# genetronhealth/uvc

Measured on AMD Instinct MI355X. Metric: pileup positions scored/sec at 300x depth, higher is better.
Workload: dtype int32

## Files before the change

### uvc_amd/csrc/uvc_device.h

```cpp
#ifndef UVC_DEVICE_H
#define UVC_DEVICE_H

#include <hip/hip_runtime.h>
#include <stdint.h>
#include "uvcgpu.h"

#define NSYM UVC_NUM_SYMBOLS
#define NBUCKETS 16
#define SQR_QUAL_DIV 32
#define MAX_INSERT_SIZE 2000
#define MAX_STR_N_BASES 100
#define UVC_MAXEV 8
#define UVC_DIGEST_MAX_VOTES (1 << 22)

enum { C_MATCH = 0, C_INS = 1, C_DEL = 2, C_REF_SKIP = 3, C_SOFT_CLIP = 4, C_HARD_CLIP = 5, C_PAD = 6, C_EQUAL = 7, C_DIFF = 8 };

struct AlnRec {
    int32_t pos, rend, mpos, isize;
    int32_t flag, mapq, dflag, l_qseq;
    int64_t seq_off;
    int64_t qbase;
    int64_t cigar_off;
    int64_t table_off;
    int64_t item_off;
    int64_t gap_off;
    int32_t n_cigar, kind;
    int32_t xm1500, go1500;
    int32_t bm1500[5];
    int32_t clip_cnt;
    int32_t nogap_penal, indel_penal;
    int32_t lclip_len, rclip_len;
    int32_t lclip_oplen, rclip_oplen;
    int32_t lclip_q;
    int32_t m_index;
    int32_t frag, fs;
    int32_t id;
    int32_t n_mutc;
    int64_t baq_pos, baq_last, baq2_last;
};

struct FastRec {
    int32_t pos, rend, qb_lo, aln;
    int32_t fmd, isize, mpos, xm1500;
    int32_t bmv, xbv, bm4c, clips;
    int32_t baq_pos, baq_last, baq2_last, ext;
};

struct FragRec {
    int32_t aln_beg, aln_end;
    int32_t beg, end;
    int32_t fs, strand, dflag, normMQ;
    int32_t n_cov, n_near;
    int32_t singleton;
    int32_t stat_kind;
};

struct FsRec {
    int32_t frag_beg, frag_end;
    int32_t beg, end;
    int32_t strand, dflag, fam, generic;
    int64_t work_off;
    int32_t l2r_end_median, r2l_end_median, nsb_min, nsb_max;
    int32_t other_fs;
    int32_t pad_;
};
static_assert(sizeof(FsRec) == 64, "k_fam_p4d fetches a unit record as four 16-byte words per lane");

struct Item { int32_t epos; uint8_t sym, flags ; uint16_t val; uint16_t dist, indel_len; int32_t pad2; };
static_assert(sizeof(Item) == 16, "Item");

struct MisItem { int32_t rank, epos, symval; };

struct FragUnit { int32_t v[12]; };
enum { UVC_FSUM_LCNT = 0 , UVC_FSUM_LTA = 5, UVC_FSUM_LTB, UVC_FSUM_LSING, UVC_FSUM_LMQ, UVC_FSUM_BDP, UVC_FSUM_BTA, UVC_FSUM_BTB, UVC_FSUM_BMQ, UVC_FSUM_N };
struct FragFast {
    int32_t beg, end, fi, flags;
    int32_t pos0, rend0, pos1, rend1;
    int32_t qb0, qb1, nogap0, nogap1;
    int32_t sq, n_cov, n_near, pad_;
    int32_t bpos0, brend0, bqb0, sp0;
    int32_t bpos1, brend1, bqb1, sp1;
};

struct AlnGap {
    int32_t epos, sym;
    int32_t len, qpos;
    int32_t weight, aln;
    int32_t mark, pad_;
};
struct GapRow { int32_t x, sym, len, ev; int64_t seq_off; int32_t cnt[8]; };
struct GapWork {
    AlnGap *ev; int32_t n_ev;
    unsigned long long *ckey, *ckey_s, *cval, *cval_s;
    unsigned long long *ikey, *ikey_s, *ival, *ival_s;
    int32_t inc_cap; int32_t *n_inc;
    GapRow *rows; int32_t *n_rows; uint8_t *seq; unsigned long long *seq_len; int64_t seq_cap;
    int32_t *maj;
    void *sort_tmp; size_t sort_tmp_bytes;
};

struct Contrib { uint8_t bsym_p1 , lmask ; uint16_t bval; uint16_t lval[8]; uint16_t pad_[2]; };
static_assert(sizeof(Contrib) == 24, "Contrib rows are zero-filled as bytes and indexed as 24-byte records");

struct HapWork { int32_t *cand, *cand_off, *cand_cap; int32_t *n_cand; unsigned long long *total; int32_t *events; };

struct DevParams { UvcParams P; };

struct RegionDev {
    int32_t beg, end; int64_t npos;
    const uint8_t *refsym;
    int32_t *rtr;
    const int64_t *baq;
    int32_t *prep32; int64_t *prep64; int32_t *thres;
    int32_t *seg32; int64_t *seg64; int32_t *vq; int32_t *bqsum;
    int32_t *frag; int32_t *fam; int32_t *faminfo32; int64_t *faminfo64; int32_t *duplex;
    int32_t *bucket;
    const uint8_t *bases; const uint8_t *quals; const uint32_t *cigars;
    const uint16_t *bq; uint32_t bq_bytes;
    AlnRec *alns; int32_t n_alns;
    int32_t n_fast;
    FastRec *frec;
    int32_t p2_off[5];
    FastRec *frec2; int32_t n_fast2; int32_t max_p2_span;
    const int32_t *complex_ids; int32_t n_complex;
    FragRec *frags; int32_t n_frags;
    int32_t *frag_nmut; int32_t *frag_mut;
    const int32_t *sweep_frags; int32_t n_sweep;
    int32_t *overflow_frags; int32_t *n_overflow;
    const int32_t *frag_sorted;
    const int32_t *frag_rank;
    int32_t frag_off[3];
    FragFast *ffast;
    FragUnit *ffast_u;
    int32_t *win; int32_t nwin;
    int32_t *fsum;
    FsRec *fss; int32_t n_fs;
    const int32_t *generic_fs; int32_t n_generic_fs; int64_t n_generic_work;
    const int32_t *generic_sorted; int32_t max_unit_span;
    uint8_t *p5flag;
    uint8_t *dirty; int32_t ndblk;
    uint32_t *occ;
    uint32_t *fam_digest;
    Contrib *table;
    int32_t *ir_list;
    Item *items; int32_t *item_cnt;
    MisItem *mis; int32_t *mis_cnt; int32_t mis_cap;
    unsigned long long *mis_total;
    int32_t max_aln_span, max_frag_span;
    int32_t any_amplicon;
    int32_t frag32;
    int32_t max_frag_depth;
    int32_t *err;
    GapWork gap;
};

#define DEV __device__ __forceinline__

DEV int imin(int a, int b) { return a < b ? a : b; }
DEV int imax(int a, int b) { return a > b ? a : b; }
DEV int64_t lmin(int64_t a, int64_t b) { return a < b ? a : b; }
DEV int64_t lmax(int64_t a, int64_t b) { return a > b ? a : b; }
DEV int64_t nnminus(int64_t a, int64_t b) { return a > b ? a - b : 0; }
DEV int ibetween(int v, int a, int b) { return imin(imax(a, v), b); }
DEV bool is_ins(int s) { return s == UVC_LINK_I3P || s == UVC_LINK_I2 || s == UVC_LINK_I1; }
DEV bool is_del(int s) { return s == UVC_LINK_D3P || s == UVC_LINK_D2 || s == UVC_LINK_D1; }
DEV bool is_subst(int s) { return s <= UVC_BASE_NN; }
DEV bool symbols_mutated(int ref, int alt) {
    if (alt <= UVC_BASE_NN) return ref != alt && ref < UVC_BASE_N && alt < UVC_BASE_N;
    return alt != UVC_LINK_M && alt != UVC_LINK_NN;
}
DEV int cig_op(uint32_t c) { return (int)(c & 0xF); }
DEV int cig_len(uint32_t c) { return (int)(c >> 4); }

#define P32(R, f, x) ((R).prep32[(size_t)(f) * (R).npos + (x)])
#define P64(R, f, x) ((R).prep64[(size_t)(f) * (R).npos + (x)])
#define TH(R, f, x) ((R).thres[(size_t)(f) * (R).npos + (x)])
#define S32(R, f, s, x) ((R).seg32[((size_t)(f) * NSYM + (s)) * (R).npos + (x)])
#define S64(R, f, s, x) ((R).seg64[((size_t)(f) * NSYM + (s)) * (R).npos + (x)])
#define VQP(R, f, s, x) ((R).vq[((size_t)(f) * NSYM + (s)) * (R).npos + (x)])
#define BQS(R, s, x) ((R).bqsum[(size_t)(s) * (R).npos + (x)])
#define FRP(R, st, f, s, x) ((R).frag[(((size_t)(st) * UVC_NFRAG + (f)) * NSYM + (s)) * (R).npos + (x)])
#define FAP(R, st, f, s, x) ((R).fam[(((size_t)(st) * UVC_NFAM + (f)) * NSYM + (s)) * (R).npos + (x)])
#define FIP(R, f, s, x) ((R).faminfo32[((size_t)(f) * NSYM + (s)) * (R).npos + (x)])
#define FI64P(R, f, s, x) ((R).faminfo64[((size_t)(f) * NSYM + (s)) * (R).npos + (x)])
#define DUP(R, f, s, x) ((R).duplex[((size_t)(f) * NSYM + (s)) * (R).npos + (x)])
#define BKP(R, st, s, b, x) ((R).bucket[((((size_t)(st) * NSYM + (s)) * NBUCKETS) + (b)) * (R).npos + (x)])
#define RTRP(R, f, x) ((R).rtr[(size_t)(f) * (R).npos + (x)])
#define BAQ1(R, p) ((R).baq[(p) - (R).beg])
#define BAQ2(R, p) ((R).baq[(R).npos + (p) - (R).beg])

DEV int cov_PREP32(const RegionDev &R, int plane, int64_t x) { return P32(R, plane, x); }
DEV int cov_FRAG(const RegionDev &R, int plane, int64_t x) {
    int v = 0;
#pragma unroll
    for (int sd = 0; sd < 2; sd++)
#pragma unroll
        for (int s = UVC_BASE_A; s <= UVC_BASE_NN; s++) v += FRP(R, sd, plane, s, x);
    return v;
}
DEV int cov_FAM(const RegionDev &R, int plane, int64_t x) {
    int v = 0;
#pragma unroll
    for (int sd = 0; sd < 2; sd++)
#pragma unroll
        for (int s = UVC_BASE_A; s <= UVC_BASE_NN; s++) v += FAP(R, sd, plane, s, x);
    return v;
}
DEV int cov_DUPLEX(const RegionDev &R, int plane, int64_t x) {
    int v = 0;
#pragma unroll
    for (int s = UVC_BASE_A; s <= UVC_BASE_NN; s++) v += DUP(R, plane, s, x);
    return v;
}

#define UVC_DIRTY_SHIFT 12
DEV bool sym_always_filled(int s) { return s < UVC_BASE_NN || s == UVC_LINK_M; }
DEV void occ_mark(const RegionDev &R, int s, int64_t x) { if (s != UVC_LINK_M && s != (int)R.refsym[x] && !((R.occ[x] >> s) & 1u)) atomicOr(&R.occ[x], 1u << s); }
DEV void mark_sym(const RegionDev &R, int s, int64_t x) { occ_mark(R, s, x); if (!sym_always_filled(s)) R.dirty[(size_t)s * R.ndblk + (x >> UVC_DIRTY_SHIFT)] = 1; }
DEV void mark_fi(const RegionDev &R, int s, int64_t x) { R.dirty[((size_t)NSYM + s) * R.ndblk + (x >> UVC_DIRTY_SHIFT)] = 1; }
DEV void mark_dup(const RegionDev &R, int s, int64_t x) { occ_mark(R, s, x); R.dirty[((size_t)2 * NSYM + s) * R.ndblk + (x >> UVC_DIRTY_SHIFT)] = 1; }

DEV void add64(int64_t *p, int64_t v) { atomicAdd((unsigned long long *)p, (unsigned long long)v); }
DEV void add_own(int32_t *p, int v) { __hip_atomic_fetch_add(p, v, __ATOMIC_RELAXED, __HIP_MEMORY_SCOPE_WORKGROUP); }
DEV void add64_own(int64_t *p, int64_t v) { __hip_atomic_fetch_add((unsigned long long *)p, (unsigned long long)v, __ATOMIC_RELAXED, __HIP_MEMORY_SCOPE_WORKGROUP); }

template <int STRIDE> struct LdsCounts {
    int *p;
    DEV int &operator[](int s) const { return p[s * STRIDE]; }
};

template <class Arr>
// ... 83 lines not shown
```

### uvc_amd/csrc/uvc_gap.hip

```cpp
#include <algorithm>
#include <cstring>
#include <hip/hip_runtime.h>
#include <rocprim/device/device_radix_sort.hpp>
#include <stdint.h>
#include "uvc_launch.h"

extern "C" size_t uvc_gap_sort_tmp_bytes(size_t n) {
    size_t bytes = 0;
    unsigned long long *k = nullptr;
    rocprim::radix_sort_pairs(nullptr, bytes, k, k, k, k, n, 0, 64, (hipStream_t)0);
    return bytes;
}

extern "C" int uvc_gap_sort(void *tmp, size_t tmp_bytes, const unsigned long long *kin, unsigned long long *kout, const unsigned long long *vin, unsigned long long *vout,
                            size_t n, int end_bit, hipStream_t s) {
    if (n == 0) return 0;
    return rocprim::radix_sort_pairs(tmp, tmp_bytes, kin, kout, vin, vout, n, 0, (unsigned)end_bit, s) == hipSuccess ? 0 : -1;
}

__global__ void __launch_bounds__(256) k_keys_pos_cls(const int32_t *pos, const int32_t *cls, int32_t beg, int shift, int64_t n, uint32_t *key, uint32_t *val) {
    const int64_t i = (int64_t)blockIdx.x * blockDim.x + threadIdx.x;
    if (i >= n) return;
    key[i] = ((uint32_t)(pos[i] - beg) | ((uint32_t)cls[i] << shift)); val[i] = (uint32_t)i;
}
__global__ void __launch_bounds__(256) k_gather4(const uint32_t *perm, int64_t n, const int32_t *a0, const int32_t *a1, const int32_t *a2, const int32_t *a3,
                                                 int32_t *o0, int32_t *o1, int32_t *o2, int32_t *o3) {
    const int64_t i = (int64_t)blockIdx.x * blockDim.x + threadIdx.x;
    if (i >= n) return;
    const int64_t j = (int64_t)perm[i];
    o0[i] = a0[j]; o1[i] = a1[j]; o2[i] = a2[j]; o3[i] = a3[j];
}
__global__ void __launch_bounds__(256) k_rank_from_sorted(const uint32_t *perm, int64_t n, int64_t n_first, int32_t *out_ids, int32_t *rank) {
    const int64_t k = (int64_t)blockIdx.x * blockDim.x + threadIdx.x;
    if (k >= n) return;
    const int32_t id = (int32_t)perm[k];
    if (out_ids && k < n_first) out_ids[k] = id;
    if (rank) rank[id] = (k < n_first ? (int32_t)k : -1);
}
extern "C" size_t uvc_sort32_tmp_bytes(size_t n) {
    size_t bytes = 0;
    uint32_t *k = nullptr;
    rocprim::radix_sort_pairs(nullptr, bytes, k, k, k, k, std::max<size_t>(n, 1), 0, 32, (hipStream_t)0);
    return bytes;
}
extern "C" int uvc_sort_by_pos_cls(const int32_t *d_pos, const int32_t *d_cls, int32_t beg, int pos_bits, int cls_bits, int64_t n, uint32_t *work , void *tmp, size_t tmp_bytes, hipStream_t s) {
    if (n <= 0) return 0;
    if (pos_bits < 1 || cls_bits < 0 || pos_bits + cls_bits > 32) return -1;
    uint32_t *key = work, *key_s = work + n, *val = work + 2 * n, *val_s = work + 3 * n;
    hipLaunchKernelGGL(k_keys_pos_cls, dim3((unsigned)((n + 255) / 256)), dim3(256), 0, s, d_pos, d_cls, beg, pos_bits, n, key, val);
    return rocprim::radix_sort_pairs(tmp, tmp_bytes, key, key_s, val, val_s, (size_t)n, 0, (unsigned)(pos_bits + cls_bits), s) == hipSuccess ? 0 : -1;
}
extern "C" void uvc_launch_gather4(const uint32_t *perm, int64_t n, const int32_t *a0, const int32_t *a1, const int32_t *a2, const int32_t *a3, int32_t *o0, int32_t *o1, int32_t *o2, int32_t *o3, hipStream_t s) {
    if (n > 0) hipLaunchKernelGGL(k_gather4, dim3((unsigned)((n + 255) / 256)), dim3(256), 0, s, perm, n, a0, a1, a2, a3, o0, o1, o2, o3);
}
extern "C" void uvc_launch_rank_from_sorted(const uint32_t *perm, int64_t n, int64_t n_first, int32_t *out_ids, int32_t *rank, hipStream_t s) {
    if (n > 0) hipLaunchKernelGGL(k_rank_from_sorted, dim3((unsigned)((n + 255) / 256)), dim3(256), 0, s, perm, n, n_first, out_ids, rank);
}

struct ColGroups { const char *base[UVC_NUM_FIELD_GROUPS]; int32_t first_col[UVC_NUM_FIELD_GROUPS + 1]; int32_t elem[UVC_NUM_FIELD_GROUPS]; };
__global__ void __launch_bounds__(256) k_gather_columns(ColGroups G, int64_t npos, const int32_t *xs, int64_t n, int32_t n_cols, long long *out) {
    const int64_t t = (int64_t)blockIdx.x * blockDim.x + threadIdx.x;
    if (t >= n * n_cols) return;
    const int64_t i = t / n_cols; const int32_t c = (int32_t)(t - i * n_cols);
    const int64_t x = xs[i];
    long long v = 0;
    if (x >= 0 && x < npos) {
        int g = 0;
        while (g + 1 < UVC_NUM_FIELD_GROUPS && c >= G.first_col[g + 1]) g++;
        const int64_t at = (int64_t)(c - G.first_col[g]) * npos + x;
        v = (G.elem[g] == 8) ? ((const long long *)G.base[g])[at] : (long long)((const int32_t *)G.base[g])[at];
    }
    out[t] = v;
}
extern "C" void uvc_launch_gather_columns(const char *const *base, const int32_t *first_col, const int32_t *elem, int64_t npos, const int32_t *d_xs, int64_t n, long long *d_out, hipStream_t s) {
    ColGroups G;
    for (int g = 0; g < UVC_NUM_FIELD_GROUPS; g++) { G.base[g] = base[g]; G.first_col[g] = first_col[g]; G.elem[g] = elem[g]; }
    G.first_col[UVC_NUM_FIELD_GROUPS] = first_col[UVC_NUM_FIELD_GROUPS];
    const int32_t n_cols = first_col[UVC_NUM_FIELD_GROUPS];
    const int64_t total = n * n_cols;
    if (total > 0) hipLaunchKernelGGL(k_gather_columns, dim3((unsigned)((total + 255) / 256)), dim3(256), 0, s, G, npos, d_xs, n, n_cols, d_out);
}
```

### uvc_amd/csrc/uvc_host.cpp

```cpp
#include "uvc_launch.h"
#include "uvc_host.h"
#include "uvc_alloc.h"
#include "uvc_prep.h"
#include "uvc_rtr.h"
#include "uvc_hap.h"
#include "uvc_cpus.h"

#include <algorithm>
#include <chrono>
#include <cmath>
#include <cstring>
#include <memory>
#include <numeric>
#include <string>
#include <thread>
#include <vector>
#define hipMalloc(p, n) uvc_dev_malloc((void **)(p), (n))
#define hipFree(p) uvc_dev_free((void *)(p))

static thread_local std::string g_err;
static int fail(int code, const std::string &msg) { g_err = msg; return code; }
template <class F> static int guarded(const char *what, F &&f) {
    try {
        const int rc = f();
// ... 237 lines not shown
    return 0;
}

static int uvcgpu_region_create_impl(uvcgpu_region_t **out, const UvcParams *params, int32_t tid, int32_t beg, int32_t end, const char *refseq) {
    if (!out || !params || !refseq || end <= beg) return fail(UVCGPU_EINVAL, "bad argument");
    if (const int rc = uvcgpu_params_check(params)) return rc;
    uvcgpu_region *r = new uvcgpu_region();
    memset(&r->prof, 0, sizeof(r->prof));
    memset(&r->R, 0, sizeof(r->R));
    r->P = *params;
    if (hipStreamCreateWithFlags(&r->stream, hipStreamNonBlocking) != hipSuccess) { delete r; return fail(UVCGPU_EDEVICE, "hipStreamCreate failed (no GPU?)"); }
    if (getenv("UVCGPU_ONE_STREAM")) {  }
    else if (hipStreamCreateWithFlags(&r->side, hipStreamNonBlocking) != hipSuccess || hipStreamCreateWithFlags(&r->side3, hipStreamNonBlocking) != hipSuccess || hipEventCreateWithFlags(&r->e_join3, hipEventDisableTiming) != hipSuccess || hipEventCreateWithFlags(&r->e_stat, hipEventDisableTiming) != hipSuccess || hipEventCreateWithFlags(&r->e_alleles, hipEventDisableTiming) != hipSuccess || hipEventCreateWithFlags(&r->e_fork, hipEventDisableTiming) != hipSuccess || hipEventCreateWithFlags(&r->e_join, hipEventDisableTiming) != hipSuccess || hipEventCreateWithFlags(&r->e_fork2, hipEventDisableTiming) != hipSuccess) {
        uvcgpu_region_destroy(r); return fail(UVCGPU_EDEVICE, "hipStreamCreate / hipEventCreate failed");
    }
    if (hipMalloc((void **)&r->R.err, 4) != hipSuccess) { uvcgpu_region_destroy(r); return fail(UVCGPU_ENOMEM, "hipMalloc failed"); }
    const int rc = configure_region(r, tid, beg, end, refseq);
    if (rc) { uvcgpu_region_destroy(r); return rc; }
    *out = r;
    return 0;
}

static int uvcgpu_region_reset_impl(uvcgpu_region_t *r, int32_t tid, int32_t beg, int32_t end, const char *refseq) {
    if (!r || !refseq || end <= beg) return fail(UVCGPU_EINVAL, "bad argument");
    if (stream_open_(r)) return fail(UVCGPU_ESTATE, "reset while a score stream is open");
    HIP_OK(hipStreamSynchronize(r->stream));
    if (r->side) HIP_OK(hipStreamSynchronize(r->side));
    if (r->side3) HIP_OK(hipStreamSynchronize(r->side3));
    free_reads(r);
    return configure_region(r, tid, beg, end, refseq);
}

static void *prep_alloc(void *ctx, size_t bytes, int zero) {
    uvcgpu_region *r = (uvcgpu_region *)ctx;
    char *p = nullptr;
    if (dev_alloc(r, bytes, &p, zero != 0)) return nullptr;
    return p;
}
static int set_reads_on_device(uvcgpu_region_t *r, const UvcReadSoA *d, bool timing, std::chrono::steady_clock::time_point t_prev) {
    auto lap = [&](const char *what) { if (!timing) return; hipStreamSynchronize(r->stream); const auto t = std::chrono::steady_clock::now();
                                       fprintf(stderr, "[uvcgpu set_reads] %-28s %8.2f ms\n", what, std::chrono::duration<double, std::milli>(t - t_prev).count()); t_prev = t; };
    const int64_t n = d->n_reads;
    if (r->npos >= ((int64_t)1 << 29)) return fail(UVCGPU_EUNSUPPORTED, "region longer than 2^29");
    if (d->n_bases >= ((int64_t)1 << 31)) return fail(UVCGPU_EUNSUPPORTED, "more than 2^31 read bases in one region: split the region");
    if (!d->bases && !d->bases4 && d->n_bases > 0) return fail(UVCGPU_EINVAL, "neither bases nor bases4");
    UvcReadSoA dd = *d;
    int32_t *d_bad = nullptr; uint16_t *bq_done = nullptr;
    if (!d->seq_off || !d->cigar_off || !d->bases) {
        int rc0;
        int64_t *so = nullptr, *co = nullptr, *b4o = nullptr; uint8_t *ub = nullptr; char *tmp = nullptr;
        const size_t tb = uvc_prep_compact_tmp_bytes(n);
        if ((rc0 = dev_alloc(r, tb, &tmp)) || (rc0 = dev_alloc(r, 1, &d_bad, true))) return rc0;
        if (!d->seq_off && (rc0 = dev_alloc(r, (size_t)n, &so))) return rc0;
        if (!d->cigar_off && (rc0 = dev_alloc(r, (size_t)n, &co))) return rc0;
        if (!d->bases && ((rc0 = dev_alloc(r, (size_t)n, &b4o)) || (rc0 = dev_alloc(r, (size_t)std::max<int64_t>(d->n_bases, 1), &ub)) || (rc0 = dev_alloc(r, (size_t)std::max<int64_t>(d->n_bases, 1), &bq_done)))) return rc0;
        const int e = uvc_prep_compact(d->l_qseq, d->n_cigar, n, d->n_bases, d->bases ? nullptr : d->bases4, d->n_bases4_bytes, d->quals, so, d->seq_off, co, b4o, ub, bq_done, d_bad, tmp, tb, r->stream);
        if (e) return fail(UVCGPU_EDEVICE, std::string("offset scans: ") + hipGetErrorString((hipError_t)e));
        if (so) dd.seq_off = so;
        if (co) dd.cigar_off = co;
        if (ub) dd.bases = ub;
        d = &dd;
    }
    UvcPrepIn in; memset(&in, 0, sizeof(in));
    in.n_reads = n; in.n_bases = d->n_bases; in.n_cigar_ops = d->n_cigar_ops; in.n_fams = d->n_fams;
    in.pos = d->pos; in.mpos = d->mpos; in.isize = d->isize; in.nm = d->nm; in.l_qseq = d->l_qseq; in.n_cigar = d->n_cigar; in.frag_id = d->frag_id; in.fam_id = d->fam_id;
    in.flag = d->flag; in.mapq = d->mapq; in.fam_strand = d->fam_strand; in.fam_dflag = d->fam_dflag; in.seq_off = d->seq_off; in.cigar_off = d->cigar_off; in.cigars = d->cigars;
    UvcPrepOut o; char msg[256];
    int rc = uvc_prep_reads(&in, &r->P, r->beg, r->end, r->npos, prep_alloc, r, r->stream, &o, msg, (int)sizeof(msg));
    if (rc) return fail(rc, msg);
    lap("nesting + CIGAR facts (device)");
    RegionDev &R = r->R;
    RawReads &W = r->W;
    W.pos = d->pos; W.endpos = o.endpos; W.mpos = d->mpos; W.isize = d->isize; W.flag = d->flag; W.mapq = d->mapq; W.nm = d->nm; W.l_qseq = d->l_qseq; W.n_cigar = d->n_cigar;
    W.frag = o.frag_of; W.fs = o.fs_of; W.dflag = o.dflag_of; W.kind = o.kind; W.seq_off = d->seq_off; W.cigar_off = d->cigar_off; W.table_off = o.table_off; W.item_off = o.item_off; W.gap_off = o.gap_off;
    R.bases = d->bases; R.quals = d->quals; R.cigars = d->cigars;
    R.frag_off[0] = 0; R.frag_off[1] = o.n_frag_strand0; R.frag_off[2] = o.n_frags;
    const int64_t n_simple = o.n_simple; const size_t nf = (size_t)o.n_frags;
    if (bq_done) { R.bq = bq_done; R.bq_bytes = (uint32_t)(d->n_bases * 2); }
    else { uint16_t *b = nullptr; if ((rc = dev_alloc(r, (size_t)std::max<int64_t>(d->n_bases, 1), &b))) return rc; R.bq = b; R.bq_bytes = (uint32_t)(d->n_bases * 2);
      if (!d_bad && (rc = dev_alloc(r, 1, &d_bad, true))) return rc;
      uvc_launch_pack_bq(R.bases, R.quals, b, d->n_bases, d_bad, r->stream); }
    { AlnRec *a; if ((rc = dev_alloc(r, (size_t)n, &a))) return rc; R.alns = a; R.n_alns = (int32_t)n; }
    R.n_fast = (int32_t)n_simple;
    { FastRec *f; if ((rc = dev_alloc(r, (size_t)n_simple, &f))) return rc; R.frec = f; }
    R.complex_ids = o.complex_ids; R.n_complex = o.n_complex;
    R.frags = o.frags; R.n_frags = o.n_frags;
    int pos_bits = 1; while (((int64_t)1 << pos_bits) < r->npos + 1) pos_bits++;
    {
        const size_t nmax = std::max<size_t>(std::max<size_t>((size_t)n, nf), 1);
        int32_t *d_rank, *d_fsorted, *d_frank; uint32_t *work; uint8_t *tmp;
        const size_t tmp_bytes = uvc_sort32_tmp_bytes(nmax);
        if ((rc = dev_alloc(r, (size_t)n, &d_rank)) || (rc = dev_alloc(r, nf, &d_fsorted)) || (rc = dev_alloc(r, nf, &d_frank)) || (rc = dev_alloc(r, 4 * nmax, &work)) || (rc = dev_alloc(r, tmp_bytes + 16, &tmp))) return rc;
        if (uvc_sort_by_pos_cls(W.pos, o.is_complex, r->beg, pos_bits, 1, n, work, tmp, tmp_bytes, r->stream) != 0) return fail(UVCGPU_EDEVICE, "device sort of the alignments failed");
        uvc_launch_rank_from_sorted(work + 3 * n, n, n_simple, nullptr, d_rank, r->stream);
        W.fast_rank = d_rank;
        if (uvc_sort_by_pos_cls(o.frag_beg, o.frag_strand, r->beg, pos_bits, 1, (int64_t)nf, work, tmp, tmp_bytes, r->stream) != 0) return fail(UVCGPU_EDEVICE, "device sort of the fragments failed");
        uvc_launch_rank_from_sorted(work + 3 * nf, (int64_t)nf, (int64_t)nf, d_fsorted, d_frank, r->stream);
        R.frag_sorted = d_fsorted; R.frag_rank = d_frank;
    }
    { FragFast *f; if ((rc = dev_alloc(r, nf, &f, true))) return rc; R.ffast = f; }
    { FragUnit *f; if ((rc = dev_alloc(r, nf, &f, true))) return rc; R.ffast_u = f; }
    R.sweep_frags = o.sweep_frags; R.n_sweep = o.n_sweep;
    { int32_t *q; if ((rc = dev_alloc(r, nf * (size_t)(UVC_MAXEV + 2) + 1, &q, true))) return rc;
      R.frag_nmut = q; R.frag_mut = q + nf; R.overflow_frags = q + nf * (size_t)(UVC_MAXEV + 1); R.n_overflow = q + nf * (size_t)(UVC_MAXEV + 2); }
    R.fss = o.fss; R.n_fs = o.n_fs;
    R.generic_fs = o.generic_fs; R.n_generic_fs = o.n_generic; R.n_generic_work = o.work;
    R.generic_sorted = o.generic_sorted; R.max_unit_span = o.max_unit_span;
    R.frag32 = (getenv("UVCGPU_FRAG32") != nullptr);
    const char *fam_path = getenv("UVCGPU_FAM_PATH");
    const bool generic_forced = (fam_path && !strcmp(fam_path, "generic"));
    R.fam_digest = nullptr;
    if (!generic_forced && o.work > 8 * r->npos && (size_t)o.work * 32 <= ((size_t)48 << 30) && o.max_unit_frags < UVC_DIGEST_MAX_VOTES) {
        uint32_t *q = nullptr; if ((rc = dev_alloc(r, (size_t)o.work * 8, &q))) return rc; R.fam_digest = q;
    }
    if (timing) fprintf(stderr, "[uvcgpu set_reads] %d fragments, %d units, %d generic units, %lld (unit, position) cells, longest unit %d, most fragments in a unit %d, %lld positions, family form %s\n",
                        o.n_frags, o.n_fs, o.n_generic, (long long)o.work, o.max_unit_span, o.max_unit_frags, (long long)r->npos, R.fam_digest ? "digest" : "generic");
    { Contrib *t; if ((rc = dev_alloc(r, (size_t)std::max<int64_t>(o.table_rows, 1), &t))) return rc; R.table = t; }
    { int32_t *t; if ((rc = dev_alloc(r, (size_t)(o.gap_slots + 2 * (int64_t)o.n_complex + 4), &t))) return rc; R.ir_list = t; }
    { Item *t; if ((rc = dev_alloc(r, (size_t)std::max<int64_t>(o.item_slots, 1), &t))) return rc; R.items = t;
      int32_t *c; if ((rc = dev_alloc(r, (size_t)o.n_complex + 1, &c, true))) return rc; R.item_cnt = c; }
    {
        const int64_t gap_slots = o.gap_slots, ins_total = o.ins_total;
        if (gap_slots >= ((int64_t)1 << 27)) return fail(UVCGPU_EUNSUPPORTED, "more than 2^27 InDel ops in one region");
        if (gap_slots > 0 && r->npos >= ((int64_t)1 << 26)) return fail(UVCGPU_EUNSUPPORTED, "region longer than 2^26 positions: split it (the InDel allele keys hold 26 position bits)");
        GapWork &G = R.gap; memset(&G, 0, sizeof(G));
        G.n_ev = (int32_t)gap_slots; G.inc_cap = (int32_t)(7 * gap_slots + 8); G.seq_cap = ins_total + 8;
        const size_t ne = (size_t)std::max<int64_t>(gap_slots, 1), ni = (size_t)G.inc_cap;
        unsigned long long *k8; int32_t *c4;
        if ((rc = dev_alloc(r, ne, &G.ev)) || (rc = dev_alloc(r, 4 * ne + 4 * ni, &k8)) || (rc = dev_alloc(r, (size_t)4, &c4, true)) || (rc = dev_alloc(r, ne, &G.rows)) || (rc = dev_alloc(r, (size_t)G.seq_cap, &G.seq)) || (rc = dev_alloc(r, 2 * ne, &G.maj))) return rc;
        G.ckey = k8; G.ckey_s = k8 + ne; G.cval = k8 + 2 * ne; G.cval_s = k8 + 3 * ne;
        G.ikey = k8 + 4 * ne; G.ikey_s = G.ikey + ni; G.ival = G.ikey + 2 * ni; G.ival_s = G.ikey + 3 * ni;
        G.n_inc = c4; G.n_rows = c4 + 1; G.seq_len = (unsigned long long *)(c4 + 2);
        G.sort_tmp_bytes = uvc_gap_sort_tmp_bytes(std::max(ne, ni));
        uint8_t *tmp; if ((rc = dev_alloc(r, G.sort_tmp_bytes + 16, &tmp))) return rc; G.sort_tmp = tmp;
    }
    { int32_t *c; if ((rc = dev_alloc(r, (size_t)4, &c, true))) return rc; R.mis_cnt = c; R.mis_total = (unsigned long long *)(c + 2); R.mis = nullptr; R.mis_cap = 0; }
    r->d_dup_units = o.dup_units; r->d_dup_off = o.dup_off; r->n_dup = o.n_dup; r->n_dup_work = o.dup_work;
    R.max_aln_span = o.max_aln_span; R.max_frag_span = o.max_frag_span;
    R.any_amplicon = o.any_amplicon;
    R.max_frag_depth = o.max_frag_depth;
    HIP_OK(hipMemsetAsync(R.table, 0, (size_t)std::max<int64_t>(o.table_rows, 1) * sizeof(Contrib), r->stream));
    lap("allocations + orders");
    uvc_launch_prelude(&R, &W, &r->P, r->stream);
    lap("prelude kernel");
    {
        const size_t np2 = (size_t)o.n_p2;
        for (int c = 0; c <= 4; c++) R.p2_off[c] = o.p2_off[c];
        uint32_t *work; uint8_t *tmp;
        const size_t tmp_bytes = uvc_sort32_tmp_bytes(std::max<size_t>(np2, 1));
        if ((rc = dev_alloc(r, 4 * np2, &work)) || (rc = dev_alloc(r, tmp_bytes + 16, &tmp))) return rc;
        for (int k = 0; k < 4; k++) if ((rc = dev_alloc(r, np2, &r->d_p2[k]))) return rc;
        if (uvc_sort_by_pos_cls(o.p2_beg, o.p2_cls, r->beg, pos_bits, 2, (int64_t)np2, work, tmp, tmp_bytes, r->stream) != 0) return fail(UVCGPU_EDEVICE, "device sort of the P2 work list failed");
        uvc_launch_gather4(work + 3 * np2, (int64_t)np2, o.p2_aln, o.p2_beg, o.p2_end, o.p2_qb, r->d_p2[0], r->d_p2[1], r->d_p2[2], r->d_p2[3], r->stream);
        { FastRec *f; if ((rc = dev_alloc(r, np2, &f))) return rc; R.frec2 = f; R.n_fast2 = (int32_t)np2; R.max_p2_span = o.max_p2_span; }
        uvc_launch_build_p2list(&R, W.fast_rank, r->d_p2[0], r->d_p2[1], r->d_p2[2], r->d_p2[3], r->stream);
    }
    HIP_OK(hipGetLastError());
    {
        unsigned long long total = 0; int32_t bad4 = 0;
        HIP_OK(hipMemcpyAsync(&total, R.mis_total, sizeof(total), hipMemcpyDeviceToHost, r->stream));
        if (d_bad) HIP_OK(hipMemcpyAsync(&bad4, d_bad, sizeof(bad4), hipMemcpyDeviceToHost, r->stream));
        HIP_OK(hipStreamSynchronize(r->stream));
        if (bad4 == 2) return fail(UVCGPU_EINVAL, "a base code outside 0..4 in UvcReadSoA::bases");
        if (bad4) return fail(UVCGPU_EINVAL, "bases4 / l_qseq / n_bases do not fit together");
        if (total > ((unsigned long long)1 << 30)) return fail(UVCGPU_EUNSUPPORTED, "more than 2^30 mismatching bases in one region");
        MisItem *q = nullptr;
        if ((rc = dev_alloc(r, (size_t)(total + 64), &q))) return rc;
        R.mis = q; R.mis_cap = (int32_t)(total + 64);
    }
    lap("P2 list sort + build");
    r->n_bases = d->n_bases;
    r->has_reads = true; r->reads_given = true;
    return 0;
}

static int uvcgpu_region_set_reads_impl(uvcgpu_region_t *r, const UvcReadSoA *in) {
    if (!r || !in) return fail(UVCGPU_EINVAL, "bad reads");
    if (stream_open_(r)) return fail(UVCGPU_ESTATE, "set_reads while a score stream is open");
    if (in->struct_size != (int32_t)sizeof(UvcReadSoA)) return fail(UVCGPU_EINVAL, "UvcReadSoA::struct_size mismatch (set it to sizeof(UvcReadSoA))");
    if (in->n_reads < 0 || in->n_fams < 0) return fail(UVCGPU_EINVAL, "bad reads");
    const bool timing = (getenv("UVCGPU_TIMING") != nullptr);
    auto t_prev = std::chrono::steady_clock::now();
    free_reads(r);
    struct SyncOnExit { hipStream_t s, s2; ~SyncOnExit() { hipStreamSynchronize(s); if (s2) hipStreamSynchronize(s2); } } sync_on_exit = { r->stream, r->side };
    const int64_t n = in->n_reads;
    if (n == 0) { r->reads_given = true; return 0; }
    if (n > INT32_MAX / 2) return fail(UVCGPU_EUNSUPPORTED, "more than 2^30 reads in one region");
    if (in->n_bases < 0 || in->n_cigar_ops < 0) return fail(UVCGPU_EINVAL, "bad reads");
    UvcReadSoA d = *in;
    int rc;
    hipStream_t small_stream = (r->side ? r->side : r->stream);
    auto up_on = [&](hipStream_t st, const void *src, size_t bytes, void **out) -> int {
        char *q = nullptr;
        int rc2 = dev_alloc(r, bytes, &q);
        if (rc2) return rc2;
        if (bytes && hipMemcpyAsync(q, src, bytes, hipMemcpyHostToDevice, st) != hipSuccess) return fail(UVCGPU_EDEVICE, "hipMemcpyAsync(H2D)");
        *out = q;
        return 0;
    };
#define UP(field, T, count) { void *q; if ((rc = up_on(small_stream, in->field, sizeof(T) * (size_t)(count), &q))) return rc; d.field = (const T *)q; }
#define UPBIG(field, T, count) { void *q; if ((rc = up_on(r->stream, in->field, sizeof(T) * (size_t)(count), &q))) return rc; d.field = (const T *)q; }
    if (in->bases) UPBIG(bases, uint8_t, in->n_bases)
    else if (in->bases4) { if (in->n_bases4_bytes < 0) return fail(UVCGPU_EINVAL, "bad reads"); UPBIG(bases4, uint8_t, in->n_bases4_bytes) }
    UPBIG(quals, uint8_t, in->n_bases)
    UP(pos, int32_t, n) UP(mpos, int32_t, n) UP(isize, int32_t, n) UP(flag, uint16_t, n) UP(mapq, uint8_t, n) UP(nm, int32_t, n) UP(l_qseq, int32_t, n)
    UP(n_cigar, int32_t, n) UP(frag_id, int32_t, n) UP(fam_id, int32_t, n) UP(fam_strand, uint8_t, n)
    if (in->seq_off) UP(seq_off, int64_t, n)
    if (in->cigar_off) UP(cigar_off, int64_t, n)
    UP(cigars, uint32_t, in->n_cigar_ops) UP(fam_dflag, uint8_t, in->n_fams)
    if (small_stream != r->stream) {
        if (hipEventRecord(r->e_fork2, small_stream) != hipSuccess || hipStreamWaitEvent(r->stream, r->e_fork2, 0) != hipSuccess) return fail(UVCGPU_EDEVICE, "hipEventRecord / hipStreamWaitEvent");
    }
#undef UPBIG
#undef UP
    if (timing) { hipStreamSynchronize(r->stream); const auto t = std::chrono::steady_clock::now(); fprintf(stderr, "[uvcgpu set_reads] %-28s %8.2f ms\n", "H2D of the columns", std::chrono::duration<double, std::milli>(t - t_prev).count()); t_prev = t; }
    return set_reads_on_device(r, &d, timing, t_prev);
}

static int uvcgpu_region_set_reads_device_impl(uvcgpu_region_t *r, const UvcReadSoA *in) {
    if (!r || !in) return fail(UVCGPU_EINVAL, "bad reads");
    if (stream_open_(r)) return fail(UVCGPU_ESTATE, "set_reads while a score stream is open");
    if (in->struct_size != (int32_t)sizeof(UvcReadSoA)) return fail(UVCGPU_EINVAL, "UvcReadSoA::struct_size mismatch (set it to sizeof(UvcReadSoA))");
    if (in->n_reads < 0 || in->n_fams < 0 || in->n_bases < 0 || in->n_cigar_ops < 0) return fail(UVCGPU_EINVAL, "bad reads");
    const bool timing = (getenv("UVCGPU_TIMING") != nullptr);
    free_reads(r);
    if (in->n_reads == 0) { r->reads_given = true; return 0; }
    if (in->n_reads > INT32_MAX / 2) return fail(UVCGPU_EUNSUPPORTED, "more than 2^30 reads in one region");
    return set_reads_on_device(r, in, timing, std::chrono::steady_clock::now());
}

static int uvcgpu_region_correct_bq_impl(uvcgpu_region_t *r) {
    if (!r) return fail(UVCGPU_EINVAL, "null region");
    if (!r->has_reads) return fail(UVCGPU_ENOREADS, "no reads");
    uvc_launch_correct_bq(&r->R, r->P.assay_sequencing_BQ_max, r->P.assay_sequencing_BQ_inc, r->stream);
    uvc_launch_pack_bq(r->R.bases, r->R.quals, (uint16_t *)r->R.bq, r->n_bases, nullptr, r->stream);
    HIP_OK(hipMemsetAsync(r->R.mis_total, 0, sizeof(unsigned long long), r->stream));
    uvc_launch_prelude(&r->R, &r->W, &r->P, r->stream);
    uvc_launch_build_p2list(&r->R, r->W.fast_rank, r->d_p2[0], r->d_p2[1], r->d_p2[2], r->d_p2[3], r->stream);
    HIP_OK(hipGetLastError());
    HIP_OK(hipStreamSynchronize(r->stream));
    r->accumulated = false;
    return 0;
}

int uvcgpu_region_read_quals(uvcgpu_region_t *r, uint8_t *dst, int64_t n) {
    if (!r || !dst) return fail(UVCGPU_EINVAL, "null argument");
    if (!r->has_reads) return fail(UVCGPU_ENOREADS, "no reads");
    if (n != r->n_bases) return fail(UVCGPU_EINVAL, "n must equal UvcReadSoA::n_bases");
    HIP_OK(hipStreamSynchronize(r->stream));
    if (n > 0) HIP_OK(hipMemcpy(dst, r->R.quals, (size_t)n, hipMemcpyDeviceToHost));
    return 0;
}

// ... 1073 lines not shown
```

### uvc_amd/csrc/uvc_kernels_acc.hip

```cpp
#include "uvc_launch.h"

DEV int wave_uniform(int v) { return __builtin_amdgcn_readfirstlane(v); }

DEV int xcd_block() {
    const int nb = gridDim.x, b = blockIdx.x, q = nb >> 3, r = nb & 7, k = b & 7, i = b >> 3;
    return k * q + (k < r ? k : r) + i;
}

DEV int bcast(int v, int j) { return __builtin_amdgcn_readlane(v, j); }
#ifdef UVC_FRAG_COARSE
#define COARSE_T(v) unsigned long long v; asm volatile("s_memtime %0\n\ts_waitcnt lgkmcnt(0)" : "=s"(v) :: "memory");
#else
#define COARSE_T(v)
#endif
DEV __amdgpu_buffer_rsrc_t bq_rsrc(const RegionDev &R) { return __builtin_amdgcn_make_buffer_rsrc((void *)R.bq, 0, (int)R.bq_bytes, 0x00020000); }
DEV int bq_load(__amdgpu_buffer_rsrc_t rs, int idx) { return (int)__builtin_amdgcn_raw_buffer_load_b16(rs, idx << 1, 0, 0); }
struct Chunk16 { int v[16]; };
DEV void load_chunk16(const FastRec *base, int kk, int hi, Chunk16 &c) {
    if (kk < hi) {
        const int4 *q = (const int4 *)(base + kk);
        const int4 a0 = q[0], a1 = q[1], a2 = q[2], a3 = q[3];
        c.v[0] = a0.x; c.v[1] = a0.y; c.v[2] = a0.z; c.v[3] = a0.w; c.v[4] = a1.x; c.v[5] = a1.y; c.v[6] = a1.z; c.v[7] = a1.w;
        c.v[8] = a2.x; c.v[9] = a2.y; c.v[10] = a2.z; c.v[11] = a2.w; c.v[12] = a3.x; c.v[13] = a3.y; c.v[14] = a3.z; c.v[15] = a3.w;
    } else {
#pragma unroll
        for (int i = 0; i < 16; i++) c.v[i] = 0;
    }
}
DEV int lower_bound_frec(const FastRec *a, int n, int key) {
    int lo = 0, hi = n;
    while (lo < hi) { int mid = (lo + hi) >> 1; if (a[mid].pos < key) lo = mid + 1; else hi = mid; }
    return lo;
}
#define WIN_LISTS 8
DEV int win_lo(const RegionDev &R, int list, int w) { return R.win[((size_t)list * 2) * R.nwin + w]; }
DEV int win_hi(const RegionDev &R, int list, int w) { return R.win[((size_t)list * 2 + 1) * R.nwin + w]; }
__global__ void __launch_bounds__(256) k_win_index(RegionDev R, int list_beg, int list_end) {
    const int64_t t = (int64_t)blockIdx.x * blockDim.x + threadIdx.x;
    const int64_t per_list = 2 * (int64_t)R.nwin;
    if (t >= per_list * (list_end - list_beg)) return;
    const int list = list_beg + (int)(t / per_list), which = (int)((t % per_list) / R.nwin), w = (int)(t % R.nwin);
    const char *base; int stride, lo, hi, span;
    if (list == 0) { base = (const char *)&R.frec[0].pos; stride = sizeof(FastRec); lo = 0; hi = R.n_fast; span = R.max_aln_span; }
    else if (list <= 4) { base = (const char *)&R.frec2[0].pos; stride = sizeof(FastRec); lo = R.p2_off[list - 1]; hi = R.p2_off[list]; span = R.max_p2_span; }
    else if (list <= 6) { base = (const char *)&R.ffast[0].beg; stride = sizeof(FragFast); lo = R.frag_off[list - 5]; hi = R.frag_off[list - 4]; span = R.max_frag_span; }
    else { base = nullptr; stride = 0; lo = 0; hi = R.n_generic_fs; span = R.max_unit_span; }
    const int w0 = R.beg + 64 * w, key = (which == 0 ? w0 - span + 1 : w0 + 64);
    if (list <= 6) { while (lo < hi) { const int mid = (lo + hi) >> 1; if (*(const int32_t *)(base + (size_t)mid * stride) < key) lo = mid + 1; else hi = mid; } }
    else { while (lo < hi) { const int mid = (lo + hi) >> 1; if (R.fss[R.generic_sorted[mid]].beg < key) lo = mid + 1; else hi = mid; } }
    R.win[((size_t)list * 2 + which) * R.nwin + w] = lo;
}
DEV int lower_bound_pos(const AlnRec *a, int n, int key) {
    int lo = 0, hi = n;
    while (lo < hi) { int mid = (lo + hi) >> 1; if (a[mid].pos < key) lo = mid + 1; else hi = mid; }
    return lo;
}

struct SegAcc {
    int s[UVC_NSEG32];
    long long l[UVC_NSEG64];
    int lp[UVC_NSEG64];
    int a1BQf, a1BQr, a2BQf, a2BQr, bq;
    DEV void zero() { for (int i = 0; i < UVC_NSEG32; i++) s[i] = 0; for (int i = 0; i < UVC_NSEG64; i++) { l[i] = 0; lp[i] = 0; } a1BQf = a1BQr = a2BQf = a2BQr = bq = 0; }
    DEV void fold() { for (int i = 0; i < UVC_NSEG64; i++) { l[i] += (long long)lp[i]; lp[i] = 0; } }
};

DEV void seg_flush(const RegionDev &R, const SegAcc &A, int sym, int64_t x) {
    mark_sym(R, sym, x);
#pragma unroll
    for (int f = 0; f < UVC_NSEG32; f++) if (A.s[f]) atomicAdd(&S32(R, f, sym, x), A.s[f]);
#pragma unroll
    for (int f = 0; f < UVC_NSEG64; f++) if (A.l[f]) add64(&S64(R, f, sym, x), A.l[f]);
    if (A.a1BQf) atomicAdd(&VQP(R, UVC_VQ_a1BQf, sym, x), A.a1BQf);
    if (A.a1BQr) atomicAdd(&VQP(R, UVC_VQ_a1BQr, sym, x), A.a1BQr);
    if (A.a2BQf) atomicAdd(&VQP(R, UVC_VQ_a2BQf, sym, x), A.a2BQf);
    if (A.a2BQr) atomicAdd(&VQP(R, UVC_VQ_a2BQr, sym, x), A.a2BQr);
    if (A.bq) atomicAdd(&BQS(R, sym, x), A.bq);
}

DEV void seg_store(const RegionDev &R, const SegAcc &A, int sym, int64_t x) {
#pragma unroll
    for (int f = 0; f < UVC_NSEG32; f++) if (A.s[f]) S32(R, f, sym, x) = A.s[f];
#pragma unroll
    for (int f = 0; f < UVC_NSEG64; f++) if (A.l[f]) S64(R, f, sym, x) = A.l[f];
    if (A.a1BQf) VQP(R, UVC_VQ_a1BQf, sym, x) = A.a1BQf;
    if (A.a1BQr) VQP(R, UVC_VQ_a1BQr, sym, x) = A.a1BQr;
    if (A.a2BQf) VQP(R, UVC_VQ_a2BQf, sym, x) = A.a2BQf;
    if (A.a2BQr) VQP(R, UVC_VQ_a2BQr, sym, x) = A.a2BQr;
    if (A.bq) BQS(R, sym, x) = A.bq;
}

struct PosThres { int t[UVC_NTHRES]; };

struct SegRead {
    int pos, rend, flag, mapq, isize, frag_pos_L, frag_pos_R, xm1500, clip_cnt, dflag;
    long long baq_pos, baq_last, baq2_last;
};

DEV SegRead make_segread(const RegionDev &R, const AlnRec &a) {
    SegRead r;
    r.pos = a.pos; r.rend = a.rend; r.flag = a.flag; r.mapq = a.mapq; r.isize = a.isize;
    r.frag_pos_L = imin(a.pos, a.mpos); r.frag_pos_R = r.frag_pos_L + abs(a.isize);
    r.xm1500 = a.xm1500; r.clip_cnt = a.clip_cnt; r.dflag = a.dflag;
    r.baq_pos = a.baq_pos; r.baq_last = a.baq_last; r.baq2_last = a.baq2_last;
    return r;
}

DEV void bidir(int &LP1, int &LP2, int &RP1, int &RP2, long long &LPL, long long &RPL, int L1, int L2, int R1, int R2, long long nl, long long nr, bool tier2, int n_indel) {
    if (nl + n_indel >= L1) LP1 += 1;
    if ((nl + n_indel >= L2) && tier2) LP2 += 1;
    if (nr >= R1) RP1 += 1;
    if ((nr >= R2) && tier2) RP2 += 1;
    LPL += nl; RPL += nr;
}

template <bool isGap>
DEV void segbias(SegAcc &A, const UvcParams &P, const SegRead &r, const PosThres &T, int rpos, long long baq_p, long long baq2_p,
                 int bq, int bm1500, int cigar_op, int indel_len, int dist_to_interfering_indel) {
    const bool is_assay_amplicon = ((r.dflag & 0x4) || ((P.primerlen > 0) && !(0x2 & P.primer_flag)));
    const bool normal_filter_primers = (P.tn_is_paired && (0x1 & P.primer_flag));
    const bool is_assay_UMI = (r.dflag & 0x1);
    const int seg_l_baq1 = (int)(baq_p - r.baq_pos + 1);
    const int _seg_r_baq = (int)(r.baq_last - baq_p + 1);
    const int seg_r_baq1 = (isGap ? (int)lmin((long long)_seg_r_baq, r.baq2_last - baq2_p + 7) : _seg_r_baq);
    const int seg_l_nbases = rpos - r.pos + 1;
    const int seg_r_nbases = r.rend - rpos;
    const bool is_high_readlen = (P.central_readlen >= P.microadjust_median_readlen_thres);
// ... 100 lines not shown
    const int min_dist2iend = ((r.flag & 0x1) ? imin(fl2, fr2) : (isrc ? r_nb : l_nb));
    const wmask m_iend = umask(!amplicon) | BAL(min_dist2iend > P.primerlen2);
    const wmask m_lp1 = BAL(l_nb >= T.t[UVC_T_aLP1t]), m_lp2 = BAL(l_nb >= T.t[UVC_T_aLP2t]);
    const wmask m_rp1 = BAL(r_nb >= T.t[UVC_T_aRP1t]), m_rp2 = BAL(r_nb >= T.t[UVC_T_aRP2t]);
    const wmask m_lb1 = BAL(l_baq >= P.bias_thres_BAQ1), m_lb2 = BAL(l_baq >= P.bias_thres_BAQ2);
    const wmask m_goodU = umask((!amplicon) || (!normal_filter_primers));
    const wmask m_goodL = m_goodU | (m_farL & m_unaffL), m_goodB = m_goodU | (m_farB & m_unaffB);
    const int d = (isrc ? fl2 : fr2);
    wmask m_i1lo, m_i1hi, m_i2lo, m_i2hi, m_nonb;
    if (isrc) {
        m_i1lo = BAL(d >= T.t[UVC_T_aLI1t]); m_i1hi = BAL(d <= T.t[UVC_T_aLI1T]); m_i2lo = BAL(d >= T.t[UVC_T_aLI2t]); m_i2hi = BAL(d <= T.t[UVC_T_aLI2T]);
        m_nonb = BAL(l_nb > r_nb);
    } else {
        m_i1lo = BAL(d >= T.t[UVC_T_aRI1t]); m_i1hi = BAL(d <= T.t[UVC_T_aRI1T]); m_i2lo = BAL(d >= T.t[UVC_T_aRI2t]); m_i2hi = BAL(d <= T.t[UVC_T_aRI2T]);
        m_nonb = BAL(l_nb < r_nb);
    }
    const wmask m_okB = umask(is_normal), m_okL = m_okB | (umask(mate_ok) & m_nonb);
    const int p2 = (is_assay_UMI || !amplicon), nc = (0 == r.clip_cnt);
    auto common = [&](SegAcc &A, int bq) {
        const int bq2 = (int)(__umul24((unsigned)bq, (unsigned)bq) / SQR_QUAL_DIV);
        if (isrc) { A.a1BQr += bq; A.a2BQr += bq2; } else { A.a1BQf += bq; A.a2BQf += bq2; }
        A.bq += bq;
        A.s[UVC_S_aMQs] += r.mapq;
        if (strand) { if (isrc) A.s[UVC_S_aDPrr] += 1; else A.s[UVC_S_aDPrf] += 1; }
        else        { if (isrc) A.s[UVC_S_aDPfr] += 1; else A.s[UVC_S_aDPff] += 1; }
        addm(A.s[UVC_S_aP3], m_p3);
        A.s[UVC_S_aNC] += nc; A.s[UVC_S_aP2] += p2;
        if (has_isize) { if (isrc) A.lp[UVC_S64_aLIT] += fl2; else A.lp[UVC_S64_aRIT] += fr2; }
    };
    auto bias = [&](SegAcc &A, bool in_all, wmask in, wmask far, wmask unaff, wmask m_rb1, wmask m_rb2, int r_baq) {
        const wmask a = (in & far), b = (in & unaff);
        addm(A.s[UVC_S_aLP1], a & m_lp1); addm(A.s[UVC_S_aLP2], a & m_lp2); addm(A.s[UVC_S_aRP1], a & m_rp1); addm(A.s[UVC_S_aRP2], a & m_rp2);
        A.s[UVC_S_aLPL] += selm(a, l_nb); A.s[UVC_S_aRPL] += selm(a, r_nb);
        addm(A.s[UVC_S_aLB1], b & m_lb1); addm(A.s[UVC_S_aLB2], b & m_lb2); addm(A.s[UVC_S_aRB1], b & m_rb1); addm(A.s[UVC_S_aRB2], b & m_rb2);
        A.lp[UVC_S64_aLBL] += selm(b, l_baq); A.lp[UVC_S64_aRBL] += selm(b, r_baq);
        if (in_all) A.s[UVC_S_aBQ2] += (in ? 1 : 0); else addm(A.s[UVC_S_aBQ2], in);
        addm(A.s[UVC_S_aP1], far & unaff & m_iend);
    };
    if (hasB) {
        common(AB, bqB);
        AB.s[UVC_S_aPF1] += amp1[imin(bqB, 255)]; AB.s[UVC_S_aPF2] += amp2[imin(bqB, 255)];
        AB.s[UVC_S_a2XM2] += xm_inc; AB.s[UVC_S_a2BM2] += bm_inc;
        bias(AB, false, BAL(bqB >= P.bias_thres_highBQ), m_farB, m_unaffB, BAL(r_baqB >= P.bias_thres_BAQ1), BAL(r_baqB >= P.bias_thres_BAQ2), r_baqB);
        if (isrc) { addm(AB.s[UVC_S_aLI1], m_i1lo & m_i1hi & m_okB); addm(AB.s[UVC_S_aLI2], m_i2lo & m_i2hi & m_okB & m_goodB); addm(AB.s[UVC_S_aLIr], m_goodB); }
        else      { addm(AB.s[UVC_S_aRI1], m_i1lo & m_i1hi & m_okB); addm(AB.s[UVC_S_aRI2], m_i2lo & m_i2hi & m_okB & m_goodB); addm(AB.s[UVC_S_aRIf], m_goodB); }
    }
    if (hasL) {
        common(AL, bqL);
        AL.s[UVC_S_aPF1] += imin(100, amp1[imin(bqL, 255)]); AL.s[UVC_S_aPF2] += imin(100, amp2[imin(bqL, 255)]);
        bias(AL, true, umask(10000 >= P.bias_thres_interfering_indel), m_farL, m_unaffL, BAL(r_baqL >= P.bias_thres_BAQ1), BAL(r_baqL >= P.bias_thres_BAQ2), r_baqL);
        if (isrc) { addm(AL.s[UVC_S_aLI1], m_i1lo & m_okL); addm(AL.s[UVC_S_aLI2], m_i2lo & m_okL & m_goodL); addm(AL.s[UVC_S_aLIr], m_goodL); }
        else      { addm(AL.s[UVC_S_aRI1], m_i1lo & m_okL); addm(AL.s[UVC_S_aRI2], m_i2lo & m_okL & m_goodL); addm(AL.s[UVC_S_aRIf], m_goodL); }
    }
}

DEV void load_thres(const RegionDev &R, PosThres &T, int64_t x) {
#pragma unroll
    for (int f = 0; f < UVC_NTHRES; f++) T.t[f] = TH(R, f, x);
}

DEV void primer_window(const UvcParams &P, const AlnRec &a, int &ibeg, int &iend) {
    const bool isrc = (a.flag & 0x10) != 0;
    ibeg = ((a.isize != 0) ? (imin(a.pos, a.mpos) + P.primerlen) : ((isrc && (0x0 == (0x1 & a.flag))) ? 0 : (a.pos + P.primerlen)));
    iend = ((a.isize != 0) ? (int)nnminus(imin(a.pos, a.mpos) + abs(a.isize), P.primerlen) : ((isrc && (0x0 == (0x1 & a.flag))) ? (int)nnminus(a.rend, P.primerlen) : INT32_MAX));
}


DEV bool has_lowbq_indel(const UvcParams &P, const AlnRec &a, const uint32_t *cigar, const uint8_t *quals) {
    auto Q = [&](int q) -> int { return (int)quals[imin(imax(q, 0), a.l_qseq - 1)]; };
    int qpos = 0;
    for (int i = 0; i < a.n_cigar; i++) {
        const int op = cig_op(cigar[i]), len = cig_len(cigar[i]);
        if (op == C_MATCH || op == C_EQUAL || op == C_DIFF || op == C_SOFT_CLIP) qpos += len;
        else if (op == C_INS) {
            for (int q2 = qpos - imin(qpos, 1); q2 < imin(qpos + len + 1, a.rend); q2++) if (Q(q2) < P.bias_thres_interfering_indel_BQ) return true;
            qpos += len;
        } else if (op == C_DEL) {
            if (imin(Q(imax(1, qpos) - 1), Q(qpos)) <= P.bias_thres_interfering_indel_BQ) return true;
        }
    }
    return false;
}

DEV void fill_fastrec(FastRec &f, const AlnRec &a, int id, int cbeg, int cend, int32_t qb_lo) {
    f.pos = cbeg; f.rend = cend; f.qb_lo = qb_lo; f.aln = id;
    f.fmd = (a.flag & 0xFFFF) | ((a.mapq & 0xFF) << 16) | ((a.dflag & 0xFF) << 24); f.isize = a.isize; f.mpos = a.mpos; f.xm1500 = a.xm1500;
    int bv[5];
    for (int s2 = 0; s2 < 5; s2++) bv[s2] = (a.bm1500[s2] > 20 ? (100 * (20 * 20) / (a.bm1500[s2] * a.bm1500[s2])) : 100);
    const int xv = (a.xm1500 > 20 ? (100 * (20 * 20) / (a.xm1500 * a.xm1500)) : 100);
    f.bmv = bv[0] | (bv[1] << 8) | (bv[2] << 16) | (bv[3] << 24); f.xbv = bv[4] | (xv << 8);
    f.bm4c = ((a.clip_cnt & 0xF) << 16) | (a.nogap_penal & 0xFFFF);
    f.clips = (a.lclip_oplen & 0xFFFF) | (a.rclip_oplen << 16);
    f.baq_pos = (int32_t)a.baq_pos; f.baq_last = (int32_t)a.baq_last; f.baq2_last = (int32_t)a.baq2_last;
    f.ext = ((cbeg - a.pos) & 0xFFFF) | ((a.rend - cend) << 16);
}

__global__ void __launch_bounds__(256) k_build_p2list(RegionDev R, const int32_t *fast_rank, const int32_t *aln, const int32_t *cbeg, const int32_t *cend, const int32_t *qb) {
    const int j = blockIdx.x * blockDim.x + threadIdx.x;
    if (j >= R.n_fast2) return;
    const int id = aln[j], rk = fast_rank[id];
    if (rk >= 0) {
        const uint4 *src = (const uint4 *)&R.frec[rk]; uint4 *dst = (uint4 *)&R.frec2[j];
        const uint4 v0 = src[0], v1 = src[1], v2 = src[2], v3 = src[3];
        dst[0] = v0; dst[1] = v1; dst[2] = v2; dst[3] = v3;
        return;
    }
    FastRec f;
    const AlnRec &a = R.alns[id];
    fill_fastrec(f, a, id, cbeg[j], (a.kind == 1 ? cbeg[j] : cend[j]), qb[j]);
    R.frec2[j] = f;
}

DEV unsigned long long load8u(const uint8_t *p) { unsigned long long v; __builtin_memcpy(&v, p, 8); return v; }
__global__ void __launch_bounds__(256) k_aln_bm(RegionDev R, RawReads W) {
    const unsigned long long K7F = 0x7F7F7F7F7F7F7F7FULL, K80 = 0x8080808080808080ULL, K01 = 0x0101010101010101ULL;
    const int sub = threadIdx.x & 7;
    for (int id = (blockIdx.x * blockDim.x + threadIdx.x) >> 3; id < R.n_alns; id += (gridDim.x * blockDim.x) >> 3) {
        const int rk = W.fast_rank[id];
        if (rk < 0) continue;
        const int pos = W.pos[id], len = W.endpos[id] - pos;
        const uint32_t c0 = R.cigars[W.cigar_off[id]];
        const uint8_t *b = R.bases + W.seq_off[id] + (cig_op(c0) == C_SOFT_CLIP ? cig_len(c0) : 0);
        const uint8_t *rf = R.refsym + (pos - R.beg);
        int cnt[5] = { 0, 0, 0, 0, 0 };
        for (int k = 8 * sub; k + 8 <= len; k += 64) {
            const unsigned long long bb = load8u(b + k), rr = load8u(rf + k);
            const unsigned long long mism = ((bb ^ rr) + K7F) & K80;
#pragma unroll
            for (int s2 = 0; s2 < 5; s2++) cnt[s2] += __popcll(mism & ~((bb ^ (K01 * (unsigned)s2)) + K7F) & K80);
        }
        { const int k = (len & ~7) + sub;
          if (k < len) { const int bs = b[k]; const bool mm = (bs != rf[k]);
#pragma unroll
                         for (int s2 = 0; s2 < 5; s2++) cnt[s2] += (mm && bs == s2); } }
#pragma unroll
        for (int s2 = 0; s2 < 5; s2++) { cnt[s2] += __shfl_xor(cnt[s2], 1); cnt[s2] += __shfl_xor(cnt[s2], 2); cnt[s2] += __shfl_xor(cnt[s2], 4); }
        if (sub == 0) {
            int32_t *dst = (int32_t *)&R.frec[rk];
#pragma unroll
            for (int s2 = 0; s2 < 5; s2++) dst[s2] = cnt[s2];
        }
    }
}

DEV int aln_prelude_one(const RegionDev &R, const RawReads &W, const UvcParams &P, const int id, AlnRec &out) {
    AlnRec a;
    a.pos = W.pos[id]; a.rend = W.endpos[id]; a.mpos = W.mpos[id]; a.isize = W.isize[id]; a.flag = W.flag[id]; a.mapq = W.mapq[id];
    a.dflag = W.dflag[id]; a.l_qseq = W.l_qseq[id]; a.seq_off = W.seq_off[id]; a.cigar_off = W.cigar_off[id]; a.table_off = W.table_off[id]; a.item_off = W.item_off[id]; a.gap_off = W.gap_off[id];
    a.n_cigar = W.n_cigar[id]; a.kind = W.kind[id]; a.frag = W.frag[id]; a.fs = W.fs[id]; a.id = id;
    const uint32_t *cigar = R.cigars + a.cigar_off;
    const uint8_t *bases = R.bases + a.seq_off;
    int nge = 0, ngo = 0, clip_cnt = 0;
    for (int i = 0; i < a.n_cigar; i++) {
        const int op = cig_op(cigar[i]);
        if (C_INS == op || C_DEL == op) { nge += cig_len(cigar[i]); ngo++; }
        if (C_SOFT_CLIP == op || C_HARD_CLIP == op) clip_cnt++;
        if (op > C_DIFF) atomicExch(R.err, UVCGPU_EUNSUPPORTED);
    }
    const int nm_cnt = (W.nm[id] >= 0 ? W.nm[id] : nge);
    const int qlen = a.rend - a.pos;
    a.xm1500 = (nm_cnt - nge) * 1500 / qlen;
    a.go1500 = ngo * 1500 / qlen;
    a.clip_cnt = clip_cnt;
    int bm[5] = { 0, 0, 0, 0, 0 };
    int qpos = 0, rpos = a.pos, lclip_q = 0, m_index = -1;
    const int rk0 = W.fast_rank[id];
    if (rk0 >= 0) {
        const int32_t *pre = (const int32_t *)&R.frec[rk0];
        for (int s2 = 0; s2 < 5; s2++) bm[s2] = pre[s2];
        for (int i = 0; i < a.n_cigar && m_index < 0; i++) {
            const int op = cig_op(cigar[i]);
            if (op == C_MATCH || op == C_EQUAL || op == C_DIFF) { m_index = i; lclip_q = qpos; }
            else if (op == C_SOFT_CLIP) qpos += cig_len(cigar[i]);
        }
    } else
    for (int i = 0; i < a.n_cigar; i++) {
        const int op = cig_op(cigar[i]), len = cig_len(cigar[i]);
        if (op == C_MATCH || op == C_EQUAL || op == C_DIFF) {
            if (m_index < 0) { m_index = i; lclip_q = qpos; }
            for (int k = 0; k < len; k++) { const int b = bases[qpos]; if (R.refsym[rpos - R.beg] != b) bm[b] += 1; qpos++; rpos++; }
        } else if (op == C_INS || op == C_SOFT_CLIP) qpos += len;
        else if (op == C_DEL || op == C_REF_SKIP) rpos += len;
    }
    for (int s = 0; s < 5; s++) a.bm1500[s] = bm[s] * 1500 / qlen;
    a.lclip_len = ((a.n_cigar > 0 && cig_op(cigar[0]) == C_SOFT_CLIP) ? cig_len(cigar[0]) : 0);
    a.rclip_len = ((a.n_cigar > 0 && cig_op(cigar[a.n_cigar - 1]) == C_SOFT_CLIP) ? cig_len(cigar[a.n_cigar - 1]) : 0);
    const int by_clip = imax(a.lclip_len, a.rclip_len) / 6;
    const int by_nm = (a.xm1500 + a.go1500) / 30;
    a.indel_penal = imin(1, by_nm + by_clip);
    a.nogap_penal = imin(4, by_nm + by_clip) + 1;
    if (by_nm + by_clip < -30000) atomicExch(R.err, UVCGPU_EUNSUPPORTED);
    a.lclip_q = lclip_q; a.m_index = m_index;
    a.lclip_oplen = 0; a.rclip_oplen = 0;
    if (a.kind == 0) {
        if (m_index > 0) a.lclip_oplen = cig_len(cigar[m_index - 1]);
        if (m_index + 1 < a.n_cigar) a.rclip_oplen = cig_len(cigar[m_index + 1]);
    }
    a.qbase = a.seq_off + lclip_q - a.pos;
    a.baq_pos = BAQ1(R, a.pos); a.baq_last = BAQ1(R, a.rend - 1); a.baq2_last = BAQ2(R, a.rend - 1);
    if (a.kind == 2 && has_lowbq_indel(P, a, cigar, R.quals + a.seq_off)) a.kind = 1;
    const int rk = W.fast_rank[id];
    int n_mis = 0;
    a.n_mutc = bm[0] + bm[1] + bm[2] + bm[3] + bm[4] + ngo;
    out = a;
    if (rk >= 0 || W.kind[id] == 2) n_mis = bm[0] + bm[1] + bm[2] + bm[3] + bm[4];
    if (rk >= 0) {
        FastRec f;
        fill_fastrec(f, a, id, a.pos, a.rend, (int32_t)(a.qbase & 0xFFFFFFFFLL));
        R.frec[rk] = f;
    }
    return n_mis;
}
__global__ void __launch_bounds__(256) k_aln_prelude(RegionDev R, RawReads W, UvcParams P) {
    static_assert(sizeof(AlnRec) % 8 == 0 && (256 * sizeof(AlnRec)) % 16 == 0, "the staged copy moves the block's records as 16-byte words");
    __shared__ __attribute__((aligned(16))) AlnRec stage[256];
    const int id0 = blockIdx.x * blockDim.x, id = id0 + threadIdx.x;
    __shared__ int mis_s[4];
    int n_mis = (id < R.n_alns) ? aln_prelude_one(R, W, P, id, stage[threadIdx.x]) : 0;
    for (int d = 32; d > 0; d >>= 1) n_mis += __shfl_xor(n_mis, d);
    if ((threadIdx.x & 63) == 0) mis_s[threadIdx.x >> 6] = n_mis;
    __syncthreads();
    if (threadIdx.x == 0) { const int t = mis_s[0] + mis_s[1] + mis_s[2] + mis_s[3]; if (t) atomicAdd(R.mis_total, (unsigned long long)t); }
    const int nrec = imin(256, R.n_alns - id0);
    if (nrec == 256) {
        const uint4 *src = (const uint4 *)&stage[0]; uint4 *dst = (uint4 *)(R.alns + id0);
        for (int i = threadIdx.x; i < (int)(256 * sizeof(AlnRec) / 16); i += 256) dst[i] = src[i];
    } else {
        const unsigned long long *src = (const unsigned long long *)&stage[0]; unsigned long long *dst = (unsigned long long *)(R.alns + id0);
        for (int i = threadIdx.x; i < nrec * (int)(sizeof(AlnRec) / 8); i += 256) dst[i] = src[i];
    }
}

DEV void snv_dnv_scatter(const RegionDev &R, const uint8_t *qbases, int q_s, int l_qseq, int apos, int rend, int s) {
    int nq = q_s, nr = s;
    int refsymbol = UVC_BASE_NN, readsymbol = UVC_NUM_SYMBOLS;
    while (refsymbol != readsymbol && nq < l_qseq && nr < rend) {
        refsymbol = R.refsym[nr - R.beg];
        readsymbol = qbases[nq];
        nq++; nr++;
    }
    if (nr == s + 2) for (int r = imax(apos, s - 1); r < imin(nr, rend); r++) atomicAdd(&P32(R, UVC_P_a_snv_dp, r - R.beg), 1);
    if (nr > s + 2)  for (int r = imax(apos, s - 1); r < imin(nr, rend); r++) atomicAdd(&P32(R, UVC_P_a_dnv_dp, r - R.beg), 1);
}

DEV void clip_event(const RegionDev &R, const UvcParams &P, int rpos, int i, int len, int pcr_dp_inc) {
    const int delta = ((0 == i) ? 0 : -1);
    if (pcr_dp_inc) {
        for (int r2 = rpos + delta - P.microadjust_near_clip_dist; r2 <= rpos + delta + P.microadjust_near_clip_dist; r2++)
            if (R.beg <= r2 && r2 < R.end) atomicAdd(&P32(R, UVC_P_a_near_pcr_clip_dp, r2 - R.beg), pcr_dp_inc);
    }
    if ((0 == pcr_dp_inc) && (len >= P.microadjust_alignment_clip_min_len)) {
        const int r2 = rpos + delta;
        if (R.beg <= r2 && r2 < R.end) atomicAdd(&P32(R, UVC_P_a_near_long_clip_dp, r2 - R.beg), 1);
    }
}

DEV int simple_base_value(const UvcParams &P, const AlnRec &a, int p, const uint8_t *quals_qbase, bool proton);

DEV void mut_event(const RegionDev &R, const UvcParams &P, const AlnRec &a, int p, int my_ref) {
    const FragRec &f = R.frags[a.frag];
    if (f.stat_kind != 0) return;
    const bool proton = (UVC_PLATFORM_IONTORRENT == P.inferred_sequencing_platform);
    int m[6] = { 0, 0, 0, 0, 0, 0 };
    int first_mis = -1;
    for (int k = f.aln_beg; k < f.aln_end; k++) {
        const AlnRec &al = R.alns[k];
        if (p < al.pos || p >= al.rend) continue;
        const int sym = R.bases[al.qbase + p];
        if (sym != my_ref && first_mis < 0) first_mis = k;
        const int v = simple_base_value(P, al, p, R.quals + al.qbase, proton);
        m[sym] = imax(m[sym], v);
    }
    if (first_mis != a.id) return;
    int cs = UVC_BASE_NN, cc = 0, ct = 0;
    for (int s2 = 0; s2 < 6; s2++) { if (cc < m[s2]) { cs = s2; cc = m[s2]; } ct += m[s2]; }
    const int con_qual = cc * 2 - ct;
    const bool highBQ = (proton ? true : (con_qual >= P.bias_thres_highBQ));
    if (symbols_mutated(my_ref, cs) && highBQ) {
        const int idx = atomicAdd(&R.frag_nmut[a.frag], 1);
        if (idx < UVC_MAXEV) R.frag_mut[(size_t)a.frag * UVC_MAXEV + idx] = p;
    }
}

#define PREPQ_CAP 192
#define PSUM_TILE 1024
enum { PS_DP = 0, PS_PCR, PS_UMI, PS_QLEN, PS_XM, PS_LIDP, PS_RIDP, PS_LIA, PS_RIA, PS_N32 };
__global__ void __launch_bounds__(256) k_prep_sums(RegionDev R, UvcParams P) {
    __shared__ int d[PS_N32][PSUM_TILE + 1];
    __shared__ unsigned long long d64[2][PSUM_TILE + 1];
    __shared__ int wtot[4];
    __shared__ unsigned long long wtot64[4];
    const int t0 = R.beg + (int)blockIdx.x * PSUM_TILE, t1 = imin(t0 + PSUM_TILE, R.beg + (int)R.npos);
    for (int i = threadIdx.x; i < PS_N32 * (PSUM_TILE + 1); i += 256) (&d[0][0])[i] = 0;
    for (int i = threadIdx.x; i < 2 * (PSUM_TILE + 1); i += 256) (&d64[0][0])[i] = 0ull;
    __syncthreads();
    const int w_first = (int)blockIdx.x * (PSUM_TILE / 64), w_last = imin(w_first + PSUM_TILE / 64, R.nwin) - 1;
    const int lo = win_lo(R, 0, w_first), hi = win_hi(R, 0, w_last);
    auto put = [&](int f, int a, int b, int v) {
        a = imax(a, t0); b = imin(b, t1);
        if (a < b && v != 0) { atomicAdd(&d[f][a - t0], v); atomicAdd(&d[f][b - t0], -v); }
    };
    auto put64 = [&](int f, int a, int b, long long v) {
        a = imax(a, t0); b = imin(b, t1);
        if (a < b && v != 0) { atomicAdd(&d64[f][a - t0], (unsigned long long)v); atomicAdd(&d64[f][b - t0], (unsigned long long)(-v)); }
    };
    for (int k = lo + (int)threadIdx.x; k < hi; k += 256) {
        const int4 *q4 = (const int4 *)(R.frec + k);
        const int4 h0 = q4[0], h1 = q4[1];
        const int apos = h0.x, rend = h0.y;
        if (rend <= t0 || apos >= t1) continue;
        const int dflag = (h1.x >> 24) & 0xFF;
        put(PS_DP, apos, rend, 1); put(PS_PCR, apos, rend, (dflag & 0x4) ? 1 : 0); put(PS_UMI, apos, rend, (dflag & 0x1) ? 1 : 0);
        put(PS_QLEN, apos, rend, rend - apos); put(PS_XM, apos, rend, h1.w);
        if (h1.y != 0) {
            const int fl = imin(apos, h1.z);
            if (h1.x & 0x10) {
                const int brk = imax(apos, imin(rend, (int)lmin((long long)fl + MAX_INSERT_SIZE, (long long)INT32_MAX)));
                put(PS_LIDP, apos, rend, 1);
                put(PS_LIA, apos, brk, 1); put64(0, apos, brk, 1LL - fl); put64(0, brk, rend, MAX_INSERT_SIZE);
            } else {
                const long long fr = (long long)fl + (long long)abs(h1.y);
                const int brk = imax(apos, imin(rend, (int)lmax(lmin(fr - MAX_INSERT_SIZE + 1, (long long)INT32_MAX), (long long)INT32_MIN)));
                put(PS_RIDP, apos, rend, 1);
                put64(1, apos, brk, MAX_INSERT_SIZE); put(PS_RIA, brk, rend, 1); put64(1, brk, rend, fr);
            }
        }
    }
    __syncthreads();
    const int lane = threadIdx.x & 63, w = threadIdx.x >> 6;
    const int n_here = t1 - t0;
    const int64_t xb = (int64_t)blockIdx.x * PSUM_TILE;
    int liA[4] = {0, 0, 0, 0}, riA[4] = {0, 0, 0, 0};
    const int plane_of[PS_N32] = { UVC_P_a_dp, UVC_P_a_pcr_dp, UVC_P_a_umi_dp, UVC_P_a_qlen, UVC_P_a_XM1500, UVC_P_a_LIDP, UVC_P_a_RIDP, -1, -1 };
    for (int f = 0; f < PS_N32; f++) {
        int v[4], run = 0;
#pragma unroll
        for (int i = 0; i < 4; i++) { run += d[f][threadIdx.x * 4 + i]; v[i] = run; }
        int inc = run;
#pragma unroll
        for (int o = 1; o < 64; o <<= 1) { const int t = __shfl_up(inc, o, 64); if (lane >= o) inc += t; }
        if (lane == 63) wtot[w] = inc;
        __syncthreads();
        int before = inc - run;
        for (int i = 0; i < w; i++) before += wtot[i];
        __syncthreads();
#pragma unroll
        for (int i = 0; i < 4; i++) {
            const int x = threadIdx.x * 4 + i, val = before + v[i];
            if (f == PS_LIA) liA[i] = val; else if (f == PS_RIA) riA[i] = val;
            else if (x < n_here && val != 0) P32(R, plane_of[f], xb + x) = val;
        }
    }
    for (int f = 0; f < 2; f++) {
        unsigned long long v[4], run = 0;
#pragma unroll
        for (int i = 0; i < 4; i++) { run += d64[f][threadIdx.x * 4 + i]; v[i] = run; }
        unsigned long long inc = run;
#pragma unroll
        for (int o = 1; o < 64; o <<= 1) { const unsigned long long t = __shfl_up(inc, o, 64); if (lane >= o) inc += t; }
        if (lane == 63) wtot64[w] = inc;
        __syncthreads();
        unsigned long long before = inc - run;
        for (int i = 0; i < w; i++) before += wtot64[i];
        __syncthreads();
#pragma unroll
        for (int i = 0; i < 4; i++) {
            const int x = threadIdx.x * 4 + i;
            const long long pp = (long long)t0 + x;
            const long long val = (long long)(before + v[i]) + (f == 0 ? pp * liA[i] : -pp * riA[i]);
            if (x < n_here && val != 0) P64(R, f == 0 ? UVC_P_a_LI : UVC_P_a_RI, xb + x) = val;
        }
    }
}

template <bool SPLIT>
__global__ void __launch_bounds__(256) k_prep_fast(RegionDev R, UvcParams P) {
    __shared__ int2 prepq[4][PREPQ_CAP];
    const int lane = threadIdx.x & 63;
    const int wave = SPLIT ? wave_uniform((int)xcd_block()) : wave_uniform((int)((xcd_block() * blockDim.x + threadIdx.x) >> 6));
    const int64_t x0 = (int64_t)wave * 64;
    if (x0 >= R.npos) return;
    const int w0 = R.beg + (int)x0;
    const int p = w0 + lane;
    const int64_t x = x0 + lane;
    const bool valid = x < R.npos;
    const int my_ref = valid ? R.refsym[x] : 0;
    const int my_baq = valid ? (int)R.baq[x] : 0;
    int ldist = 0, rdist = 0, hbq = 0;
    long long lbaq = 0, rbaq = 0;
    const int lo = wave_uniform(win_lo(R, 0, (int)(x0 >> 6))), hi = wave_uniform(win_hi(R, 0, (int)(x0 >> 6)));
    COARSE_T(ct1)
    const __amdgpu_buffer_rsrc_t rs = bq_rsrc(R);
    int2 *myq = prepq[threadIdx.x >> 6];
    int nq = 0;
    auto drain = [&]() {
        for (int i = lane; i < nq; i += 64) {
            const int2 e = myq[i];
            const AlnRec &a = R.alns[e.x];
            snv_dnv_scatter(R, R.bases + a.seq_off, (int)(a.qbase + e.y - a.seq_off), a.l_qseq, a.pos, a.rend, e.y);
            mut_event(R, P, a, e.y, R.refsym[e.y - R.beg]);
        }
        nq = 0;
    };
    for (int k0 = lo + (SPLIT ? 64 * (int)(threadIdx.x >> 6) : 0); k0 < hi; k0 += (SPLIT ? 256 : 64)) {
        Chunk16 c;
        load_chunk16(R.frec, k0 + lane, hi, c);
        const int n = imin(64, hi - k0);
        auto fetch = [&](int j) { return bq_load(rs, bcast(c.v[2], j) + p); };
        auto one = [&](int j, int bqn) {
            const int b = bqn & 0xFF, q = (bqn >> 8) & 0xFF;
            const int apos = bcast(c.v[0], j), rend = bcast(c.v[1], j);
            if (rend <= w0) return;
            const bool cover = (valid && p >= apos && p < rend);
            const wmask mm = BAL(cover && b != my_ref);
            if (mm) {
                if (nq > PREPQ_CAP - 64) drain();
                if (cover && b != my_ref) myq[nq + (int)__builtin_popcountll(mm & ((1ull << lane) - 1ull))] = make_int2(bcast(c.v[3], j), p);
                nq += (int)__builtin_popcountll(mm);
            }
            if (cover) {
                if (q >= P.bias_thres_highBQ) {
                    ldist += p - apos + 1; rdist += rend - p;
                    lbaq += (my_baq - bcast(c.v[12], j) + 1);
                    rbaq += (bcast(c.v[13], j) - my_baq + 1);
                    hbq += 1;
                }
                const int clips = bcast(c.v[11], j);
                if (clips != 0) {
                    const int lclip = clips & 0xFFFF, rclip = (clips >> 16) & 0xFFFF;
                    const int pcr_inc = (((bcast(c.v[4], j) >> 24) & 0x4) ? 1 : 0);
                    if (p == apos && lclip > 0) clip_event(R, P, apos, 0, lclip, pcr_inc);
                    if (p == rend - 1 && rclip > 0) clip_event(R, P, rend, 1, rclip, pcr_inc);
                }
            }
        };
        int r0 = fetch(0), r1 = (1 < n ? fetch(1) : 0), r2 = (2 < n ? fetch(2) : 0), r3 = (3 < n ? fetch(3) : 0);
        for (int j = 0; j < n; j += 4) {
            { const int v = r0; if (j + 4 < n) r0 = fetch(j + 4); one(j, v); }
            if (j + 1 < n) { const int v = r1; if (j + 5 < n) r1 = fetch(j + 5); one(j + 1, v); }
            if (j + 2 < n) { const int v = r2; if (j + 6 < n) r2 = fetch(j + 6); one(j + 2, v); }
            if (j + 3 < n) { const int v = r3; if (j + 7 < n) r3 = fetch(j + 7); one(j + 3, v); }
        }
    }
    if (nq > 0) drain();
    COARSE_T(ct2)
    if (!valid) return;
    if (hbq) {
        atomicAdd(&P32(R, UVC_P_a_highBQ_dp, x), hbq);
        atomicAdd(&P32(R, UVC_P_a_l_dist_sum, x), ldist); atomicAdd(&P32(R, UVC_P_a_r_dist_sum, x), rdist);
        add64(&P64(R, UVC_P_a_l_BAQ_sum, x), lbaq); add64(&P64(R, UVC_P_a_r_BAQ_sum, x), rbaq);
    }
#ifdef UVC_FRAG_COARSE
    asm volatile("s_waitcnt vmcnt(0)" ::: "memory");
    COARSE_T(ct3)
    if (lane == 0 && ((int)(x0 >> 6) % 2999) == 7) printf("coarse prep wave %d lists %llu epilogue %llu\n", (int)(x0 >> 6), ct2 - ct1, ct3 - ct2);
#endif
}

__global__ void __launch_bounds__(64) k_prep_slow(RegionDev R, UvcParams P) {
    const int t = blockIdx.x, lane = threadIdx.x;
    if (t >= R.n_complex) return;
    const AlnRec &a = R.alns[R.complex_ids[t]];
    const uint32_t *cigar = R.cigars + a.cigar_off;
    const uint8_t *bases = R.bases + a.seq_off, *quals = R.quals + a.seq_off;
    const int off = R.beg, rend = a.rend, apos = a.pos, n_cigar = a.n_cigar;
    const long long baq_last = R.end - 1;
    int nge = 0, ngo = 0, insbaq_sum = 0, delbaq_sum = 0, inslen_sum = 0, dellen_sum = 0;
    int qpos = 0, rpos = apos;
    for (int i = 0; i < n_cigar; i++) {
        const int op = cig_op(cigar[i]), len = cig_len(cigar[i]);
        if (C_INS == op) { nge += len; ngo++; insbaq_sum += (int)(BAQ1(R, lmin((long long)rpos + len, baq_last)) - BAQ1(R, rpos)); inslen_sum += len; qpos += len; }
        else if (C_DEL == op) { nge += len; ngo++; delbaq_sum += (int)(BAQ1(R, lmin((long long)rpos + len, baq_last)) - BAQ1(R, rpos)); dellen_sum += len; rpos += len; }
        else if (op == C_MATCH || op == C_EQUAL || op == C_DIFF) { qpos += len; rpos += len; }
        else if (op == C_REF_SKIP) rpos += len;
        else if (op == C_SOFT_CLIP) qpos += len;
    }
    const int qlen = rend - apos;
    const int xm1500 = a.xm1500, go1500 = a.go1500;
    const int avg_gaplen = nge / imax(1, ngo);
    const int frag_pos_L = imin(apos, a.mpos), frag_pos_R = frag_pos_L + abs(a.isize);
    const bool isrc = (a.flag & 0x10) != 0;
    const int pcr_dp_inc = ((a.dflag & 0x4) ? 1 : 0), umi_dp_inc = ((a.dflag & 0x1) ? 1 : 0);
    const int atd = P.indel_adj_tracklen_dist;
    const int nrtr = (int)R.npos;
    const int isize = a.isize, l_qseq = a.l_qseq;
    const long long baq_apos = BAQ1(R, apos), baq_rlast = BAQ1(R, rend - 1);
    qpos = 0; rpos = apos;
    for (int i = 0; i < n_cigar; i++) {
        const int op = cig_op(cigar[i]), len = cig_len(cigar[i]);
        if (op == C_MATCH || op == C_EQUAL || op == C_DIFF) {
            for (int j = lane; j < len; j += 64) {
                const int rp = rpos + j, qp = qpos + j;
                const int64_t x = rp - off;
                if (pcr_dp_inc) atomicAdd(&P32(R, UVC_P_a_pcr_dp, x), pcr_dp_inc);
                if (umi_dp_inc) atomicAdd(&P32(R, UVC_P_a_umi_dp, x), umi_dp_inc);
                atomicAdd(&P32(R, UVC_P_a_dp, x), 1);
                atomicAdd(&P32(R, UVC_P_a_qlen, x), qlen);
                atomicAdd(&P32(R, UVC_P_a_XM1500, x), xm1500);
                atomicAdd(&P32(R, UVC_P_a_GO1500, x), go1500);
                atomicAdd(&P32(R, UVC_P_a_GAPLEN, x), avg_gaplen);
                if (isize != 0) {
                    if (isrc) { add64(&P64(R, UVC_P_a_LI, x), imin(rp - frag_pos_L + 1, MAX_INSERT_SIZE)); atomicAdd(&P32(R, UVC_P_a_LIDP, x), 1); }
                    else      { add64(&P64(R, UVC_P_a_RI, x), imin(frag_pos_R - rp, MAX_INSERT_SIZE));     atomicAdd(&P32(R, UVC_P_a_RIDP, x), 1); }
                }
                snv_dnv_scatter(R, bases, qp, l_qseq, apos, rend, rp);
                if (quals[qp] >= P.bias_thres_highBQ) {
                    atomicAdd(&P32(R, UVC_P_a_l_dist_sum, x), rp - apos + 1);
                    atomicAdd(&P32(R, UVC_P_a_r_dist_sum, x), rend - rp);
                    atomicAdd(&P32(R, UVC_P_a_inslen_sum, x), inslen_sum);
                    atomicAdd(&P32(R, UVC_P_a_dellen_sum, x), dellen_sum);
                    add64(&P64(R, UVC_P_a_l_BAQ_sum, x), (int)(BAQ1(R, rp) - baq_apos + 1));
                    add64(&P64(R, UVC_P_a_r_BAQ_sum, x), (int)(baq_rlast - BAQ1(R, rp) + 1));
                    add64(&P64(R, UVC_P_a_insBAQ_sum, x), insbaq_sum);
                    add64(&P64(R, UVC_P_a_delBAQ_sum, x), delbaq_sum);
                    atomicAdd(&P32(R, UVC_P_a_highBQ_dp, x), 1);
                }
            }
            qpos += len; rpos += len;
        } else if (op == C_INS || op == C_DEL) {
            const int i1 = imax(atd, rpos - off) - atd, i2 = imin(rpos - off + atd, nrtr - 1);
            const int t1 = RTRP(R, UVC_RTR_tracklen, i1), t2 = RTRP(R, UVC_RTR_tracklen, i2);
            const int unitlen2 = imax(1, (t1 > t2) ? RTRP(R, UVC_RTR_unitlen, i1) : RTRP(R, UVC_RTR_unitlen, i2));
            const int rtr_lo = imax((off + RTRP(R, UVC_RTR_begpos, i1)) - atd, apos);
            const int rtr_hi = imin((off + RTRP(R, UVC_RTR_begpos, i2) + t2) + atd, rend);
            const int inv100 = (int)(100u / ((0 == (unsigned)len % (unsigned)unitlen2) ? ((unsigned)len / (unsigned)unitlen2) : 4u));
// ... 2521 lines not shown
    if (zp.fam >= 0 && !dirty[((size_t)zp.fam * NSYM + zp.sym) * ndblk + b]) return;
    const int64_t x0 = (int64_t)b << UVC_DIRTY_SHIFT, x1 = (x0 + ((int64_t)1 << UVC_DIRTY_SHIFT) < npos ? x0 + ((int64_t)1 << UVC_DIRTY_SHIFT) : npos);
    char *p0 = slab + zp.off + x0 * zp.elem, *p1 = slab + zp.off + x1 * zp.elem;
    char *a0 = (char *)(((uintptr_t)p0 + 15) & ~(uintptr_t)15), *a1 = (char *)((uintptr_t)p1 & ~(uintptr_t)15);
    if (a0 >= a1) { for (char *q = p0 + threadIdx.x; q < p1; q += 256) *q = 0; return; }
    for (char *q = p0 + threadIdx.x; q < a0; q += 256) *q = 0;
    const uint4 z = make_uint4(0u, 0u, 0u, 0u);
    for (uint4 *q = (uint4 *)a0 + threadIdx.x; q < (uint4 *)a1; q += 256) *q = z;
    for (char *q = a1 + threadIdx.x; q < p1; q += 256) *q = 0;
}
extern "C" void uvc_launch_zero_state(char *slab, const ZeroPlane *planes, int n_planes, uint8_t *dirty, int ndblk, int64_t npos, hipStream_t s) {
    if (n_planes <= 0 || ndblk <= 0) return;
    hipLaunchKernelGGL(k_zero_state, dim3((unsigned)n_planes, (unsigned)ndblk), dim3(256), 0, s, slab, planes, dirty, ndblk, npos);
}
__global__ void __launch_bounds__(256) k_check_dirty(RegionDev R, unsigned long long *n_bad) {
    const int64_t x = (int64_t)blockIdx.x * blockDim.x + threadIdx.x;
    const int s = (int)blockIdx.y;
    if (x >= R.npos) return;
    const int b = (int)(x >> UVC_DIRTY_SHIFT);
    long long core = 0, fi = 0, du = 0;
    for (int f = 0; f < UVC_NSEG32; f++) core |= S32(R, f, s, x);
    for (int f = 0; f < UVC_NSEG64; f++) core |= S64(R, f, s, x);
    for (int f = 0; f < UVC_NVQ; f++) core |= VQP(R, f, s, x);
    core |= BQS(R, s, x);
    for (int st = 0; st < 2; st++) { for (int f = 0; f < UVC_NFRAG; f++) core |= FRP(R, st, f, s, x); for (int f = 0; f < UVC_NFAM; f++) core |= FAP(R, st, f, s, x); }
    for (int f = 0; f < UVC_NFAMINFO32; f++) fi |= FIP(R, f, s, x);
    for (int f = 0; f < UVC_NFAMINFO64; f++) fi |= FI64P(R, f, s, x);
    for (int f = 0; f < UVC_NDUPLEX; f++) du |= DUP(R, f, s, x);
    int bad = 0;
    if (core && !sym_always_filled(s) && !R.dirty[(size_t)s * R.ndblk + b]) bad++;
    if (fi && !R.dirty[((size_t)NSYM + s) * R.ndblk + b]) bad++;
    if (du && !R.dirty[((size_t)2 * NSYM + s) * R.ndblk + b]) bad++;
    if (bad) atomicAdd(n_bad, (unsigned long long)bad);
}
extern "C" void uvc_launch_check_dirty(const RegionDev *R, unsigned long long *d_n_bad, hipStream_t s) {
    hipLaunchKernelGGL(k_check_dirty, dim3((unsigned)((R->npos + 255) / 256), NSYM), dim3(256), 0, s, *R, d_n_bad);
}

struct AccForms { bool vcf, proton, split_windows, p2_plain, frag_plain, h16, fam, digest, duplex; int n_gen; };
static AccForms acc_forms(const RegionDev *R, const UvcParams *P, int n_dup) {
    AccForms F;
    F.vcf = (P->inferred_is_vcf_generated != 0);
    F.proton = (UVC_PLATFORM_IONTORRENT == P->inferred_sequencing_platform);
    const char *sp_env = getenv("UVCGPU_SPLIT");
    const long long per_window = (long long)R->n_fast2 * (R->max_p2_span + 64) / (R->npos > 0 ? R->npos : 1);
    F.split_windows = sp_env ? (atoi(sp_env) != 0) : (R->nwin < 4 * 1024 && per_window >= 1024);
    F.p2_plain = !F.proton && !R->any_amplicon && !(P->primerlen > 0 && !(0x2 & P->primer_flag)) && (P->central_readlen >= P->microadjust_median_readlen_thres);
    F.frag_plain = F.vcf && !F.proton && !(0x1 & P->fam_flag) && !(P->microadjust_padded_deletion_flag & 0x1);
    F.h16 = (R->max_frag_depth < 65536) && !R->frag32;
    F.fam = (R->n_generic_fs > 0);
    F.digest = (R->fam_digest != nullptr);
    F.duplex = F.fam && F.vcf && n_dup;
    F.n_gen = F.proton ? R->n_frags : R->n_sweep;
    return F;
}
static void print_forms(const AccForms &F) {
    fprintf(stderr, "[uvcgpu accumulate] forms prep=%s p2=%s%s frag=%s,%s,%s family=%s duplex=%s frag_generic=%s\n",
            !F.vcf ? "none" : F.split_windows ? "split" : "wave",
            !F.vcf ? "none" : F.split_windows ? "split" : "wave", !F.vcf ? "" : F.p2_plain ? ",plain" : ",generic",
            F.h16 ? "h16" : "b32", (F.split_windows && F.h16) ? "split" : "wave", F.frag_plain ? "plain" : "generic",
            !F.fam ? "none" : F.digest ? "digest" : "generic",
            !F.duplex ? "none" : F.digest ? "digest" : "generic",
            !F.n_gen ? "none" : F.proton ? "all" : "sweep");
}
template <bool DO_L, bool DO_B>
static void launch_p2_fast(const char *kname, const AccForms &F, const RegionDev *R, const UvcParams *P, unsigned nwin, UvcProf *prof, hipStream_t s) {
    if (F.split_windows && F.p2_plain) TIMED(prof, kname, hipLaunchKernelGGL((k_p2_fast_split<DO_L, DO_B, true>), dim3(R->nwin), dim3(256), 0, s, *R, *P));
    else if (F.split_windows) TIMED(prof, kname, hipLaunchKernelGGL((k_p2_fast_split<DO_L, DO_B, false>), dim3(R->nwin), dim3(256), 0, s, *R, *P));
    else if (F.p2_plain) TIMED(prof, kname, hipLaunchKernelGGL((k_p2_fast<DO_L, DO_B, true>), dim3(nwin), dim3(256), 0, s, *R, *P));
    else TIMED(prof, kname, hipLaunchKernelGGL((k_p2_fast<DO_L, DO_B, false>), dim3(nwin), dim3(256), 0, s, *R, *P));
}

extern "C" void uvc_launch_accumulate(const RegionDev *R, const UvcParams *P, int half_ratio_phred, const int32_t *dup_units, int n_dup, const int64_t *dup_off, int64_t n_dup_work,
                                      const UvcAccStreams *st, UvcProf *prof) {
    const hipStream_t s = st->s, side = st->side, side3 = st->side3;
    const hipEvent_t e_fork = st->e_fork, e_join = st->e_join, e_fork2 = st->e_fork2, e_join3 = st->e_join3, e_stat = st->e_stat, e_alleles = st->e_alleles;
    const unsigned nwin = nblk(R->npos, 256);
    const AccForms F = acc_forms(R, P, n_dup);
    if (getenv("UVCGPU_TIMING")) print_forms(F);
    if (prof) prof->n = 0;
    hipStream_t s2 = (side ? side : s);
    hipStream_t s3 = ((side && side3) ? side3 : s2);
    {
        const int64_t n = 2 * (int64_t)R->nwin * 5;
        TIMED(prof, "k_win_index", hipLaunchKernelGGL(k_win_index, dim3(nblk(n, 256)), dim3(256), 0, s, *R, 0, 5));
        if (R->n_generic_fs) hipLaunchKernelGGL(k_win_index, dim3(nblk(2 * (int64_t)R->nwin, 256)), dim3(256), 0, s, *R, 7, 8);
    }
    if (P->inferred_is_vcf_generated && R->n_fast) TIMED(prof, "k_prep_sums", hipLaunchKernelGGL(k_prep_sums, dim3(nblk(R->npos, PSUM_TILE)), dim3(256), 0, s, *R, *P));
    if (P->inferred_is_vcf_generated) {
        if (side && R->n_complex) { hipEventRecord(e_fork, s); hipStreamWaitEvent(s2, e_fork, 0); }
        if (R->n_complex) TIMED2(prof, "k_prep_slow", hipLaunchKernelGGL(k_prep_slow, dim3(R->n_complex), dim3(64), 0, s, *R, *P));
        if (side && R->n_complex) hipEventRecord(e_join, s2);
        if (F.split_windows) TIMED(prof, "k_prep_fast", hipLaunchKernelGGL(k_prep_fast<true>, dim3(R->nwin), dim3(256), 0, s, *R, *P));
        else TIMED(prof, "k_prep_fast", hipLaunchKernelGGL(k_prep_fast<false>, dim3(nwin), dim3(256), 0, s, *R, *P));
        if (side && R->n_complex) hipStreamWaitEvent(s, e_join, 0);
    }
    if (P->inferred_is_vcf_generated) TIMED(prof, "k_thres", hipLaunchKernelGGL(k_thres, dim3(nblk(R->npos, 256)), dim3(256), 0, s, *R, *P, half_ratio_phred));
    if (side) { hipEventRecord(e_fork, s); hipStreamWaitEvent(s2, e_fork, 0); if (s3 != s2) hipStreamWaitEvent(s3, e_fork, 0); }
    if (P->inferred_is_vcf_generated && R->n_complex) TIMED2(prof, "k_p2_slow_walk", hipLaunchKernelGGL(k_p2_slow<true>, dim3(nblk(R->n_complex, 64)), dim3(64), 0, s, *R, *P));
    if (R->n_complex) TIMED3(prof, "k_p2_slow_table", hipLaunchKernelGGL(k_p2_slow<false>, dim3(nblk(R->n_complex, 64)), dim3(64), 0, s, *R, *P));
    TIMED3(prof, "k_fragstat_fast", hipLaunchKernelGGL(k_fragstat_fast, dim3(nblk(R->n_frags, 256)), dim3(256), 0, s, *R, *P));
    TIMED3(prof, "k_win_index_frag", hipLaunchKernelGGL(k_win_index, dim3(nblk(2 * (int64_t)R->nwin * 2, 256)), dim3(256), 0, s, *R, 5, 7));
    if (R->n_sweep) TIMED3(prof, "k_fragstat_sweep", hipLaunchKernelGGL(k_fragstat_sweep, dim3(R->n_sweep), dim3(64), 0, s, *R, *P, R->sweep_frags, (const int32_t *)nullptr, R->n_sweep));
    TIMED3(prof, "k_fragstat_overflow", hipLaunchKernelGGL(k_fragstat_sweep, dim3(imin_h(R->n_frags, 65535)), dim3(64), 0, s, *R, *P, (const int32_t *)R->overflow_frags, (const int32_t *)R->n_overflow, 0));
    if (UVC_PLATFORM_IONTORRENT != P->inferred_sequencing_platform)
        TIMED3(prof, "k_frag_sums", hipLaunchKernelGGL(k_frag_sums, dim3(nblk(R->npos, FSUM_TILE), 2), dim3(256), 0, s, *R, *P));
    if (P->inferred_is_vcf_generated) {
        launch_p2_fast<false, true>("k_p2_fast_base", F, R, P, nwin, prof, s);
        if (side) { hipEventRecord(e_fork2, s); hipStreamWaitEvent(s3, e_fork2, 0); }
        TIMED3(prof, "k_p2_mism", hipLaunchKernelGGL(k_p2_mism, dim3(2048), dim3(256), 0, s, *R, *P));
        launch_p2_fast<true, false>("k_p2_fast_link", F, R, P, nwin, prof, s);
    }
    if (side) {
        hipEventRecord(e_join, s2); hipStreamWaitEvent(s, e_join, 0);
        if (s3 != s2) { hipEventRecord(e_join3, s3); hipStreamWaitEvent(s, e_join3, 0); hipStreamWaitEvent(s2, e_join3, 0); }
    }
    const GapWork &G = R->gap;
    hipMemsetAsync(G.n_inc, 0, 16, s2);
    if (P->inferred_is_vcf_generated && G.n_ev > 0) {
        TIMED2(prof, "k_gap", {
            hipLaunchKernelGGL(k_gap_keys, dim3(nblk(G.n_ev, 256)), dim3(256), 0, s, *R);
            uvc_gap_sort(G.sort_tmp, G.sort_tmp_bytes, G.ckey, G.ckey_s, G.cval, G.cval_s, (size_t)G.n_ev, 58, s);
            hipMemsetAsync(G.ikey, 0xFF, sizeof(unsigned long long) * (size_t)G.inc_cap, s);
            hipLaunchKernelGGL(k_gap_alleles, dim3(nblk(G.n_ev, 64)), dim3(64), 0, s, *R, *P);
            if (side) hipEventRecord(e_alleles, s);
            uvc_gap_sort(G.sort_tmp, G.sort_tmp_bytes, G.ikey, G.ikey_s, G.ival, G.ival_s, (size_t)G.inc_cap, 64, s);
            hipLaunchKernelGGL(k_gap_rows, dim3(nblk(G.inc_cap, 256)), dim3(256), 0, s, *R);
            hipLaunchKernelGGL(k_gap_rows_add, dim3(nblk(G.inc_cap, 256)), dim3(256), 0, s, *R);
            hipLaunchKernelGGL(k_gap_rows_fin, dim3(nblk(G.n_ev, 256)), dim3(256), 0, s, *R);
        });
    }
    if (side && !(P->inferred_is_vcf_generated && G.n_ev > 0)) hipEventRecord(e_alleles, s2);
    if (R->n_generic_fs) TIMED3(prof, "k_fam_stat", hipLaunchKernelGGL(k_fam_stat, dim3(nblk(R->n_generic_fs, 64)), dim3(64), 0, s, *R, *P));
    if (side) { hipEventRecord(e_stat, s3); hipEventRecord(e_fork2, s2); }
    if (P->inferred_is_vcf_generated && R->n_complex) TIMED(prof, "k_p2_items", hipLaunchKernelGGL(k_p2_items, dim3(R->n_complex), dim3(64), 0, s, *R, *P));
    {
        if (F.n_gen) TIMED(prof, "k_frag_generic", hipLaunchKernelGGL(k_frag_generic, dim3(imin_h(F.n_gen, 1 << 20), imin_h((R->max_frag_span + 63) / 64, 16)), dim3(64), 0, s, *R, *P, F.proton ? (const int32_t *)nullptr : R->sweep_frags, F.n_gen));
    }
    {
        const bool plain = F.frag_plain;
        if (F.split_windows && F.h16 && plain) TIMED(prof, "k_frag", hipLaunchKernelGGL(k_frag16_split<true>, dim3(R->nwin), dim3(256), 0, s, *R, *P));
        else if (F.split_windows && F.h16) TIMED(prof, "k_frag", hipLaunchKernelGGL(k_frag16_split<false>, dim3(R->nwin), dim3(256), 0, s, *R, *P));
        else if (plain && F.h16) TIMED(prof, "k_frag", hipLaunchKernelGGL(k_frag16<true>, dim3(nwin), dim3(256), 0, s, *R, *P));
        else if (plain) TIMED(prof, "k_frag", hipLaunchKernelGGL(k_frag<true>, dim3(nwin), dim3(256), 0, s, *R, *P));
        else if (F.h16) TIMED(prof, "k_frag", hipLaunchKernelGGL(k_frag16<false>, dim3(nwin), dim3(256), 0, s, *R, *P));
        else TIMED(prof, "k_frag", hipLaunchKernelGGL(k_frag<false>, dim3(nwin), dim3(256), 0, s, *R, *P));
    }
    if (R->n_generic_fs) {
        if (side) { hipStreamWaitEvent(s, e_stat, 0); hipStreamWaitEvent(s, e_alleles, 0); }
        if (F.digest) TIMED(prof, "k_fam_p4", { hipLaunchKernelGGL(k_fam_p4d, dim3(nblk(R->npos, 64)), dim3(256), 0, s, *R, *P);
                                               hipLaunchKernelGGL(k_fam_p4d_rest, dim3(R->n_generic_fs), dim3(64), 0, s, *R, *P); });
        else TIMED(prof, "k_fam_p4", hipLaunchKernelGGL(k_fam_p4, dim3(nblk(R->n_generic_work, 256)), dim3(256), 0, s, *R, *P));
        if (P->inferred_is_vcf_generated) {
            if (F.digest) TIMED(prof, "k_fam_p5", hipLaunchKernelGGL(k_fam_p5d, dim3(nblk(R->npos, 64)), dim3(256), 0, s, *R, *P));
            else TIMED(prof, "k_fam_p5", hipLaunchKernelGGL(k_fam_p5, dim3(nblk(R->n_generic_work, 256)), dim3(256), 0, s, *R, *P));
            if (F.duplex && F.digest) TIMED(prof, "k_duplex", hipLaunchKernelGGL(k_duplex_d, dim3(n_dup), dim3(64), 0, s, *R, dup_units, n_dup, dup_off, n_dup_work));
            else if (F.duplex) TIMED(prof, "k_duplex", hipLaunchKernelGGL(k_duplex, dim3(nblk(n_dup_work, 256)), dim3(256), 0, s, *R, *P, dup_units, n_dup, dup_off, n_dup_work));
        }
    }
    if (P->inferred_is_vcf_generated) TIMED(prof, "k_p5b", hipLaunchKernelGGL(k_p5b, dim3(nblk(R->npos * 2, 256)), dim3(256), 0, s, *R, *P));
    if (side) hipStreamWaitEvent(s, e_fork2, 0);
}
```

### uvc_amd/csrc/uvc_launch.h

```cpp
#ifndef UVC_LAUNCH_H
#define UVC_LAUNCH_H
#include "uvc_device.h"

struct RawReads {
    const int32_t *pos, *endpos, *mpos, *isize, *nm, *l_qseq, *n_cigar, *frag, *fs, *dflag, *kind, *fast_rank;
    const uint16_t *flag; const uint8_t *mapq;
    const int64_t *seq_off, *cigar_off, *table_off, *item_off, *gap_off;
};
static_assert(sizeof(RawReads) == 19 * sizeof(void *), "RawReads is 19 device pointers");
struct UvcProf { int on; int n; const char *name[32]; hipEvent_t ev[32][2]; };
static inline int uvc_prof_begin(UvcProf *p, const char *name, hipStream_t s) {
    if (!p || !p->on || p->n >= 32) return -1;
    const int i = p->n++;
    p->name[i] = name;
    if (!p->ev[i][0]) { hipEventCreate(&p->ev[i][0]); hipEventCreate(&p->ev[i][1]); }
    hipEventRecord(p->ev[i][0], s);
    return i;
}
static inline void uvc_prof_end(UvcProf *p, int i, hipStream_t s) { if (i >= 0) hipEventRecord(p->ev[i][1], s); }
struct ZeroPlane { unsigned long long off; int32_t elem; int16_t fam, sym; };
static_assert(sizeof(ZeroPlane) == 16, "the host uploads the plane table as 16-byte rows");
struct UvcScoreRangeDev { int beg, end, first, flags; };
static_assert(sizeof(UvcScoreRangeDev) == 16, "the host uploads the range table as 16-byte rows");
struct UvcRangeRow { int x0, first; };
static_assert(sizeof(UvcRangeRow) == 8, "the host uploads the range table as 8-byte rows");
struct UvcRangeCursor { int rid = -1, first = 0, next = 0, x0 = 0; };
DEV void uvc_range_find(UvcRangeCursor &g, const UvcRangeRow *tab, int n_ranges, long long i) {
    if (i >= g.first && i < g.next) return;
    int lo = 0, hi = n_ranges;
    while (hi - lo > 1) { const int mid = (lo + hi) >> 1; if (tab[mid].first <= i) lo = mid; else hi = mid; }
    g.rid = lo; g.first = tab[lo].first; g.x0 = tab[lo].x0; g.next = tab[lo + 1].first;
}
struct UvcUnitSpan { int lo, hi; };
static_assert(sizeof(UvcUnitSpan) == 8, "the host sizes the span scratch as 8-byte rows");

struct UvcScoreIn {
    const RegionDev *R; const UvcParams *P; const UvcScoreRequest *req;
    const UvcIndelAllele *alleles; const int32_t *allele_rows; int64_t n_alleles;
    const UvcGapRow *gap_rows; const uint8_t *gap_seq; const UvcTumorKey *tkeys;
    char *scratch; const int32_t *force_sites;
    const UvcScoreRangeDev *ranges; int64_t n_ranges, n_compact;
};
struct UvcAccStreams { hipStream_t s, side, side3; hipEvent_t e_fork, e_join, e_fork2, e_join3, e_stat, e_alleles; };

extern "C" {
void uvc_launch_correct_bq(const RegionDev *R, int bq_max, int bq_inc, hipStream_t s);
void uvc_launch_pack_bq(const uint8_t *bases, const uint8_t *quals, uint16_t *bq, int64_t n, int32_t *bad, hipStream_t s);
void uvc_launch_build_p2list(const RegionDev *R, const int32_t *fast_rank, const int32_t *aln, const int32_t *cbeg, const int32_t *cend, const int32_t *qb, hipStream_t s);
void uvc_launch_prelude(const RegionDev *R, const RawReads *W, const UvcParams *P, hipStream_t s);
void uvc_launch_zero_state(char *slab, const ZeroPlane *planes, int n_planes, uint8_t *dirty, int ndblk, int64_t npos, hipStream_t s);
void uvc_launch_check_dirty(const RegionDev *R, unsigned long long *d_n_bad, hipStream_t s);
void uvc_launch_accumulate(const RegionDev *R, const UvcParams *P, int half_ratio_phred, const int32_t *dup_units, int n_dup, const int64_t *dup_off, int64_t n_dup_work,
                           const UvcAccStreams *st, UvcProf *prof);
void uvc_launch_hap_cand(const RegionDev *R, const HapWork *H, int units, hipStream_t s);
void uvc_launch_hap_events(const RegionDev *R, const UvcParams *P, const HapWork *H, int units, int n_cand, hipStream_t s);
int uvc_launch_score(const UvcScoreIn *in, int32_t *d_fields, int64_t capacity, int32_t *d_fields_kept, hipStream_t s);
size_t uvc_score_scratch_bytes(int64_t npos_scored, int64_t capacity);
size_t uvc_score_scratch_zero_bytes(int64_t npos_scored, int64_t capacity);
int uvc_launch_score_gate(const UvcScoreIn *in, int64_t chunk_records, int64_t tab_cap, hipStream_t s);
int uvc_launch_score_chunk(const UvcScoreIn *in, char *set, int64_t chunk_records, int with_kept, int64_t win_g, int64_t win_n, int64_t win_groups, int64_t win_records, hipStream_t s);
size_t uvc_score_set_bytes(int64_t chunk_records, int64_t ngroups, int with_kept);
size_t uvc_score_set_bytes_per_record(void);
int32_t *uvc_score_set_fields(char *set, int64_t chunk_records, int64_t ngroups, int kept);
size_t uvc_score_stream_pos_bytes(int64_t npos_scored, int64_t tab_cap);
size_t uvc_score_stream_table_offset(int64_t npos_scored);
void uvc_launch_check_presence(const RegionDev *R, unsigned long long *d_n_bad, hipStream_t s);
void uvc_launch_block_stats(const RegionDev *R, const UvcParams *P, int64_t x0, int64_t n, int32_t *d_out, hipStream_t s);
void uvc_launch_block_stats_windows(const RegionDev *R, const UvcParams *P, const long long *d_win, int n_win, int64_t n, int32_t *d_out, hipStream_t s);
void uvc_launch_coverage(const RegionDev *R, const UvcRangeRow *d_tab, int n_ranges, int64_t n_total, const int32_t *thr, int n_thr, long long *d_out, long long *d_scratch, int64_t scratch_rows, hipStream_t s);
const char *uvc_coverage_name(int id);
int64_t uvc_coverage_scratch_rows(int n_ranges, int64_t n_total);
void uvc_launch_errprofile(const RegionDev *R, const UvcRangeRow *d_tab, int n_ranges, int64_t n_total, int min_depth, int max_alt_permille, long long *d_out, long long *d_scratch, hipStream_t s);
const char *uvc_errprofile_level_name(int id);
int64_t uvc_errprofile_scratch_cells(void);
void uvc_launch_famstats(const RegionDev *R, const int32_t *pos, const int32_t *endpos, const int32_t *fs_of, UvcUnitSpan *d_span, const UvcFamilyRange *d_ranges, int n_ranges, long long *d_rows, hipStream_t s);
const char *uvc_famstats_name(int id);
void uvc_launch_readprofile_depth(const RegionDev *R, const RawReads *W, int64_t n_bases, int min_mapq, int32_t *d_dx, int32_t *d_x, int32_t *d_scratch, hipStream_t s);
void uvc_launch_readprofile_status(const RegionDev *R, const UvcRangeRow *d_tab, int n_ranges, int min_depth, int max_alt_permille, int32_t *d_dx, const int32_t *d_x, uint8_t *d_status,
                                   long long *d_parts, int32_t *d_scratch, hipStream_t s);
void uvc_launch_readprofile_bin(const RegionDev *R, const RawReads *W, int64_t n_bases, int min_mapq, const uint8_t *d_status, long long *d_parts, long long *d_out, const int32_t *d_scratch, hipStream_t s);
const char *uvc_readprofile_class_name(int c);
int64_t uvc_readprofile_copies(void);
int64_t uvc_readprofile_scratch_ints(int64_t n_alns, int64_t npos);
void uvc_launch_callable_count(const RegionDev *R, const UvcRangeRow *d_tab, int n_ranges, int64_t n_total, const UvcCallableRequest *req, unsigned char *d_mask, int *d_blocks, hipStream_t s);
void uvc_launch_callable_emit(const RegionDev *R, const UvcRangeRow *d_tab, int n_ranges, int64_t n_total, const unsigned char *d_mask, const int *d_blocks, UvcCallableRun *d_runs, hipStream_t s);
int64_t uvc_callable_blocks(int64_t n_total);
const char *uvc_callable_name(int bit);
size_t uvc_gap_sort_tmp_bytes(size_t n);
int uvc_gap_sort(void *tmp, size_t tmp_bytes, const unsigned long long *kin, unsigned long long *kout, const unsigned long long *vin, unsigned long long *vout, size_t n, int end_bit, hipStream_t s);
size_t uvc_sort32_tmp_bytes(size_t n);
int uvc_sort_by_pos_cls(const int32_t *d_pos, const int32_t *d_cls, int32_t beg, int pos_bits, int cls_bits, int64_t n, uint32_t *work , void *tmp, size_t tmp_bytes, hipStream_t s);
void uvc_launch_gather4(const uint32_t *perm, int64_t n, const int32_t *a0, const int32_t *a1, const int32_t *a2, const int32_t *a3, int32_t *o0, int32_t *o1, int32_t *o2, int32_t *o3, hipStream_t s);
void uvc_launch_rank_from_sorted(const uint32_t *perm, int64_t n, int64_t n_first, int32_t *out_ids, int32_t *rank, hipStream_t s);
void uvc_launch_gather_columns(const char *const *base, const int32_t *first_col, const int32_t *elem, int64_t npos, const int32_t *d_xs, int64_t n, long long *d_out, hipStream_t s);
size_t uvc_prep_compact_tmp_bytes(int64_t n);
int uvc_prep_compact(const int32_t *l_qseq, const int32_t *n_cigar, int64_t n, int64_t n_bases, const uint8_t *bases4, int64_t n_b4, const uint8_t *quals, int64_t *seq_off_out, const int64_t *seq_off_in,
                     int64_t *cigar_off_out, int64_t *b4_off, uint8_t *bases_out, uint16_t *bq_out, int32_t *bad, void *tmp, size_t tmp_bytes, hipStream_t s);
}
#endif
```

### uvc_amd/csrc/uvc_prep.h

```cpp
#ifndef UVC_PREP_H
#define UVC_PREP_H
#include "uvc_device.h"

struct UvcPrepIn {
    int64_t n_reads, n_bases, n_cigar_ops; int32_t n_fams;
    const int32_t *pos, *mpos, *isize, *nm, *l_qseq, *n_cigar, *frag_id, *fam_id;
    const uint16_t *flag; const uint8_t *mapq, *fam_strand, *fam_dflag;
    const int64_t *seq_off, *cigar_off;
    const uint32_t *cigars;
};
struct UvcPrepOut {
    int32_t *endpos, *kind, *dflag_of, *frag_of, *fs_of, *p2_first, *complex_ids, *is_complex;
    int32_t *frag_beg, *frag_strand;
    int64_t *table_off, *item_off, *gap_off;
    FragRec *frags; FsRec *fss;
    int32_t *generic_fs, *generic_sorted, *sweep_frags, *dup_units; int64_t *dup_off;
    int32_t *p2_aln, *p2_beg, *p2_end, *p2_qb, *p2_cls;
    int32_t n_frags, n_fs, n_complex, n_simple, n_generic, n_dup, n_sweep, n_frag_strand0;
    int32_t max_aln_span, max_frag_span, max_unit_span, max_unit_frags, max_p2_span, max_frag_depth, any_amplicon;
    int32_t p2_off[5];
    int64_t n_p2, table_rows, item_slots, gap_slots, ins_total, work, dup_work;
};
typedef void *(*UvcPrepAlloc)(void *ctx, size_t bytes, int zero);
extern "C" int uvc_prep_reads(const UvcPrepIn *in, const UvcParams *P, int32_t rbeg, int32_t rend, int64_t npos, UvcPrepAlloc alloc, void *ctx, hipStream_t s,
                              UvcPrepOut *out, char *errmsg, int errcap);
#endif
```

### uvc_amd/csrc/uvc_prep.hip

```cpp
#include <algorithm>
#include <cstdio>
#include <cstring>
#include <hip/hip_runtime.h>
#include <stdint.h>
#include "uvc_prep.h"
#include "uvc_launch.h"

namespace {
#define PDEV __device__ __forceinline__
PDEV int pmin(int a, int b) { return a < b ? a : b; }
PDEV int pmax(int a, int b) { return a > b ? a : b; }
enum { PC_MATCH = 0, PC_INS = 1, PC_DEL = 2, PC_REF_SKIP = 3, PC_SOFT_CLIP = 4, PC_HARD_CLIP = 5, PC_PAD = 6, PC_EQUAL = 7, PC_DIFF = 8 };
PDEV bool is_m(int op) { return op == PC_MATCH || op == PC_EQUAL || op == PC_DIFF; }
PDEV int wave_max(int v) { for (int d = 32; d > 0; d >>= 1) v = pmax(v, __shfl_xor(v, d)); return v; }
PDEV int wave_sum(int v) { for (int d = 32; d > 0; d >>= 1) v += __shfl_xor(v, d); return v; }

#define SC_BLOCK 256
#define SC_ITEMS 8
#define SC_TILE (SC_BLOCK * SC_ITEMS)
PDEV long long wave_sum64(long long v) { for (int d = 32; d > 0; d >>= 1) v += __shfl_xor(v, d); return v; }
template <int NC> PDEV void block_sums(long long (&v)[NC], long long (*sh)[NC] ) {
    const int wv = threadIdx.x >> 6;
#pragma unroll
    for (int c = 0; c < NC; c++) v[c] = wave_sum64(v[c]);
    if ((threadIdx.x & 63) == 0) { for (int c = 0; c < NC; c++) sh[wv][c] = v[c]; }
    __syncthreads();
    if (threadIdx.x == 0) { for (int c = 0; c < NC; c++) v[c] = sh[0][c] + sh[1][c] + sh[2][c] + sh[3][c]; }
}
template <int NC> __global__ void __launch_bounds__(1024) k_tile_tops(long long *tile_sums, int ntiles, long long *totals) {
    __shared__ long long sh[1024];
    for (int c = 0; c < NC; c++) {
        long long carry = 0;
        for (int b0 = 0; b0 < ntiles; b0 += 1024) {
            const int i = b0 + (int)threadIdx.x;
            const long long v = (i < ntiles ? tile_sums[(size_t)c * ntiles + i] : 0);
            sh[threadIdx.x] = v;
            __syncthreads();
            for (int d = 1; d < 1024; d <<= 1) {
                const long long o = (threadIdx.x >= (unsigned)d ? sh[threadIdx.x - d] : 0);
                __syncthreads();
                sh[threadIdx.x] += o;
                __syncthreads();
            }
            if (i < ntiles) tile_sums[(size_t)c * ntiles + i] = carry + sh[threadIdx.x] - v;
            const long long tot = sh[1023];
            __syncthreads();
            carry += tot;
        }
        if (threadIdx.x == 0) totals[c] = carry;
    }
}
template <int NC> PDEV void block_excl(long long (&v)[NC], const long long *tile_pref , int ntiles, int tile, long long (*shw)[NC] ) {
    const int lane = threadIdx.x & 63, wv = threadIdx.x >> 6;
    long long inc[NC];
#pragma unroll
    for (int c = 0; c < NC; c++) {
        inc[c] = v[c];
        for (int d = 1; d < 64; d <<= 1) { const long long o = __shfl_up(inc[c], d); if (lane >= d) inc[c] += o; }
    }
    if (lane == 63) { for (int c = 0; c < NC; c++) shw[wv][c] = inc[c]; }
    __syncthreads();
#pragma unroll
    for (int c = 0; c < NC; c++) {
        long long base = tile_pref[(size_t)c * ntiles + tile];
        for (int q = 0; q < 4; q++) if (q < wv) base += shw[q][c];
        v[c] = base + inc[c] - v[c];
    }
}

struct ScanCols { const void *in[3]; void *out[3]; int64_t n[3]; int in64[3], out64[3], inclusive[3]; };
PDEV long long col_load(const ScanCols &C, int c, int64_t i) { return i < C.n[c] ? (C.in64[c] ? ((const long long *)C.in[c])[i] : (long long)((const int32_t *)C.in[c])[i]) : 0LL; }
__global__ void __launch_bounds__(SC_BLOCK) k_cols_sums(ScanCols C, long long *tile_sums, int ntiles) {
    __shared__ long long sh[4][3];
    long long v[3] = { 0, 0, 0 };
    for (int k = 0; k < SC_ITEMS; k++) {
        const int64_t i = (int64_t)blockIdx.x * SC_TILE + (int64_t)k * SC_BLOCK + threadIdx.x;
#pragma unroll
        for (int c = 0; c < 3; c++) v[c] += col_load(C, c, i);
    }
    block_sums<3>(v, sh);
    if (threadIdx.x == 0) { for (int c = 0; c < 3; c++) tile_sums[(size_t)c * ntiles + blockIdx.x] = v[c]; }
}
__global__ void __launch_bounds__(SC_BLOCK) k_cols_apply(ScanCols C, const long long *tile_pref, int ntiles) {
    __shared__ long long shw[4][3];
    const int64_t i0 = (int64_t)blockIdx.x * SC_TILE + (int64_t)threadIdx.x * SC_ITEMS;
    long long e[3][SC_ITEMS], v[3] = { 0, 0, 0 };
#pragma unroll
    for (int c = 0; c < 3; c++) { for (int k = 0; k < SC_ITEMS; k++) { e[c][k] = col_load(C, c, i0 + k); v[c] += e[c][k]; } }
    block_excl<3>(v, tile_pref, ntiles, (int)blockIdx.x, shw);
#pragma unroll
    for (int c = 0; c < 3; c++) {
        for (int k = 0; k < SC_ITEMS; k++) {
            const int64_t i = i0 + k;
            if (i >= C.n[c]) break;
            const long long o = (C.inclusive[c] ? v[c] + e[c][k] : v[c]);
            if (C.out64[c]) ((long long *)C.out[c])[i] = o; else ((int32_t *)C.out[c])[i] = (int32_t)o;
            v[c] += e[c][k];
        }
    }
}

struct Stage1 {
    int32_t err, max_aln_span, n_frags, n_fs, n_complex, any_amplicon;
    int32_t p2_cls[4]; int32_t max_p2_span, pad_;
    int64_t n_p2, table_rows, item_slots, gap_slots, ins_total;
};
struct Stage2 {
    int32_t err, max_frag_span, max_unit_span, max_unit_frags, n_generic, n_dup, n_sweep, n_frag_strand0, max_frag_depth, pad_;
    int64_t work, dup_work;
};

__global__ void __launch_bounds__(256) k_read_facts(UvcPrepIn in, int32_t rbeg, int32_t rend, int seg_eligible,
                                                    int32_t *endpos, int32_t *kind, int32_t *dflag_of, int32_t *new_frag, int32_t *new_fs, int32_t *is_complex,
                                                    int32_t *n_p2, int64_t *gaps, int64_t *trows, int64_t *items, int64_t *ins, Stage1 *T, long long *tile_sums, int ntiles) {
    int w_err = 0, w_span = 0, w_p2span = 0, w_cls[4] = { 0, 0, 0, 0 }, w_amp = 0;
    long long col[8] = { 0, 0, 0, 0, 0, 0, 0, 0 };
    for (int k8 = 0; k8 < SC_ITEMS; k8++) {
    const int64_t i = (int64_t)blockIdx.x * SC_TILE + (int64_t)k8 * SC_BLOCK + threadIdx.x;
    if (i >= in.n_reads) break;
    const int32_t nc = in.n_cigar[i], lq = in.l_qseq[i], pos = in.pos[i];
    int32_t o_end = pos + 1, o_kind = 1, o_np2 = 0; int64_t o_gaps = 0, o_trows = 0, o_items = 0, o_ins = 0;
    int err = 0;
    const int fam = in.fam_id[i], strand = in.fam_strand[i];
    const bool bad_fam = (fam < 0 || fam >= in.n_fams || strand < 0 || strand > 1);
    if (bad_fam) err = 5;
    if (in.seq_off[i] < 0 || in.seq_off[i] + lq > in.n_bases || in.cigar_off[i] < 0 || in.cigar_off[i] + nc > in.n_cigar_ops || nc < 1) err = 1;
    if (!err) {
        const uint32_t *cg = in.cigars + in.cigar_off[i];
        int32_t e = pos; int64_t q = 0, del_total = 0; int n_m = 0; bool simple = true;
        for (int k = 0; k < nc; k++) {
            const int op = (int)(cg[k] & 0xF); const int32_t len = (int32_t)(cg[k] >> 4);
            if (op > PC_DIFF) { err = 2; break; }
            if (is_m(op) || op == PC_DEL || op == PC_REF_SKIP) e += len;
            if (is_m(op) || op == PC_INS || op == PC_SOFT_CLIP) q += len;
            if (is_m(op)) n_m++;
            else if (!(op == PC_SOFT_CLIP || op == PC_HARD_CLIP)) simple = false;
            if (op == PC_INS || op == PC_DEL) o_gaps++;
            if (op == PC_INS) o_ins += len;
            if (op == PC_DEL) del_total += len;
        }
        if (!err) {
            if (e == pos) e = pos + 1;
            if (q != lq) err = 3;
        }
        if (!err) {
            if (n_m != 1 || nc > 3) simple = false;
            if (simple && nc == 3) { const int o0 = cg[0] & 0xF, o2 = cg[2] & 0xF; if (is_m(o0) || is_m(o2)) simple = false; }
            if (pos < rbeg || e > rend - 1) err = 4;
        }
        if (!err) {
            bool ok = simple || seg_eligible;
            int32_t rp = pos, np2 = 0, span = 1;
            for (int k = 0; k < nc && ok; k++) {
                const int op = (int)(cg[k] & 0xF); const int32_t len = (int32_t)(cg[k] >> 4);
                if (is_m(op)) { if (rp - pos > 65535 || e - (rp + len) > 65535) ok = false; np2++; span = pmax(span, len); rp += len; }
                else if (op == PC_DEL) rp += len;
                else if (op == PC_INS || op == PC_SOFT_CLIP || op == PC_HARD_CLIP) {}
                else ok = false;
            }
            o_end = e; o_np2 = (ok ? np2 : 0);
            o_kind = simple ? 0 : (ok ? 2 : 1);
            if (!simple) { o_trows = (e - pos) + 1; o_items = 2 * (int64_t)lq + 2 * del_total + nc + 4; }
            else { o_gaps = 0; o_ins = 0; w_span = pmax(w_span, e - pos); }
            if (o_np2) {
                const int fl = in.flag[i];
                const int cls = ((fl & 0x10) ? 1 : 0) | ((((fl & 0x81) == 0x81) ? ((fl & 0x20) != 0) : ((fl & 0x10) != 0)) ? 2 : 0);
                w_cls[0] += (cls == 0) * o_np2; w_cls[1] += (cls == 1) * o_np2; w_cls[2] += (cls == 2) * o_np2; w_cls[3] += (cls == 3) * o_np2; w_p2span = pmax(w_p2span, span);
            }
        }
    }
    if (err) { w_err = pmax(w_err, err); o_kind = 1; o_gaps = 0; o_ins = 0; o_np2 = 0; }
    endpos[i] = o_end; kind[i] = o_kind; n_p2[i] = o_np2; gaps[i] = o_gaps; trows[i] = o_trows; items[i] = o_items; ins[i] = o_ins; is_complex[i] = (o_kind != 0);
    const bool ok_fam = !bad_fam;
    const int df = ok_fam ? (int)in.fam_dflag[fam] : 0;
    dflag_of[i] = df;
    if (df & 0x4) w_amp = 1;
    const bool nfs = (i == 0) || in.fam_id[i - 1] != fam || in.fam_strand[i - 1] != strand;
    const bool nfr = (nfs || in.frag_id[i - 1] != in.frag_id[i]);
    new_fs[i] = nfs; new_frag[i] = nfr;
    col[0] += nfr; col[1] += nfs; col[2] += (o_kind != 0); col[3] += o_np2; col[4] += o_trows; col[5] += o_items; col[6] += o_ins; col[7] += o_gaps;
    }
    {
        __shared__ long long shc[4][8];
        block_sums<8>(col, shc);
        if (threadIdx.x == 0) { for (int c = 0; c < 8; c++) tile_sums[(size_t)c * ntiles + blockIdx.x] = col[c]; }
    }
    __shared__ int sh[4][8];
    w_err = wave_max(w_err); w_span = wave_max(w_span); w_p2span = wave_max(w_p2span); w_amp = wave_max(w_amp);
    for (int c = 0; c < 4; c++) w_cls[c] = wave_sum(w_cls[c]);
    const int wv = threadIdx.x >> 6;
    if ((threadIdx.x & 63) == 0) { sh[wv][0] = w_err; sh[wv][1] = w_span; sh[wv][2] = w_p2span; sh[wv][3] = w_amp; for (int c = 0; c < 4; c++) sh[wv][4 + c] = w_cls[c]; }
    __syncthreads();
    if (threadIdx.x == 0) {
        int v[8];
        for (int q = 0; q < 8; q++) { v[q] = sh[0][q]; for (int w = 1; w < 4; w++) v[q] = (q < 4 ? pmax(v[q], sh[w][q]) : v[q] + sh[w][q]); }
        if (v[0]) atomicMax(&T->err, v[0]);
        if (v[1]) atomicMax(&T->max_aln_span, v[1]);
        if (v[2]) atomicMax(&T->max_p2_span, v[2]);
        if (v[3]) T->any_amplicon = 1;
        for (int c = 0; c < 4; c++) if (v[4 + c]) atomicAdd(&T->p2_cls[c], v[4 + c]);
    }
}

__global__ void __launch_bounds__(SC_BLOCK) k_facts_apply(int64_t n, const long long *tile_pref, int ntiles, const long long *totals, const int32_t *kind, const int32_t *new_frag, const int32_t *new_fs,
                                                          const int32_t *n_p2, const int64_t *trows, const int64_t *items, const int64_t *gaps,
                                                          int32_t *frag_of, int32_t *fs_of, int32_t *p2_first, int64_t *table_off, int64_t *item_off, int64_t *gap_off, int32_t *complex_ids, Stage1 *T) {
    __shared__ long long shw[4][7];
    const int64_t i0 = (int64_t)blockIdx.x * SC_TILE + (int64_t)threadIdx.x * SC_ITEMS;
    long long v[7] = { 0, 0, 0, 0, 0, 0, 0 };
    int e_nf[SC_ITEMS], e_ns[SC_ITEMS], e_k[SC_ITEMS], e_p2[SC_ITEMS]; long long e_tr[SC_ITEMS], e_it[SC_ITEMS], e_gp[SC_ITEMS];
#pragma unroll
    for (int k = 0; k < SC_ITEMS; k++) {
        const int64_t i = i0 + k; const bool in = (i < n);
        e_nf[k] = in ? new_frag[i] : 0; e_ns[k] = in ? new_fs[i] : 0; e_k[k] = in ? kind[i] : 0; e_p2[k] = in ? n_p2[i] : 0;
        e_tr[k] = in ? trows[i] : 0; e_it[k] = in ? items[i] : 0; e_gp[k] = in ? gaps[i] : 0;
        v[0] += e_nf[k]; v[1] += e_ns[k]; v[2] += (e_k[k] != 0); v[3] += e_p2[k]; v[4] += e_tr[k]; v[5] += e_it[k]; v[6] += e_gp[k];
    }
    {
        const int lane = threadIdx.x & 63, wv = threadIdx.x >> 6;
        long long inc[7];
#pragma unroll
        for (int c = 0; c < 7; c++) { inc[c] = v[c]; for (int d = 1; d < 64; d <<= 1) { const long long o = __shfl_up(inc[c], d); if (lane >= d) inc[c] += o; } }
        if (lane == 63) { for (int c = 0; c < 7; c++) shw[wv][c] = inc[c]; }
        __syncthreads();
#pragma unroll
        for (int c = 0; c < 7; c++) {
            long long base = tile_pref[(size_t)(c < 6 ? c : 7) * ntiles + blockIdx.x];
            for (int q = 0; q < 4; q++) if (q < wv) base += shw[q][c];
            v[c] = base + inc[c] - v[c];
        }
    }
#pragma unroll
    for (int k = 0; k < SC_ITEMS; k++) {
        const int64_t i = i0 + k;
        if (i >= n) break;
        v[0] += e_nf[k]; v[1] += e_ns[k];
        frag_of[i] = (int32_t)v[0] - 1; fs_of[i] = (int32_t)v[1] - 1;
        p2_first[i] = (int32_t)v[3];
        if (e_k[k] == 0) { table_off[i] = -1; item_off[i] = -1; gap_off[i] = -1; }
        else { table_off[i] = v[4]; item_off[i] = v[5]; gap_off[i] = v[6]; complex_ids[v[2]] = (int32_t)i; }
        v[2] += (e_k[k] != 0); v[3] += e_p2[k]; v[4] += e_tr[k]; v[5] += e_it[k]; v[6] += e_gp[k];
    }
    if (blockIdx.x == 0 && threadIdx.x == 0) {
        T->n_frags = (int32_t)totals[0]; T->n_fs = (int32_t)totals[1]; T->n_complex = (int32_t)totals[2];
        T->n_p2 = totals[3]; T->table_rows = totals[4]; T->item_slots = totals[5]; T->ins_total = totals[6]; T->gap_slots = totals[7];
    }
}

__global__ void __launch_bounds__(256) k_mark_first(UvcPrepIn in, const int32_t *new_frag, const int32_t *new_fs, const int32_t *frag_of, const int32_t *fs_of,
                                                    int32_t *frag_first, int32_t *fs_first_frag, int32_t *fam_fs, int32_t n_frags, int32_t n_fs, Stage2 *T) {
    const int64_t i = (int64_t)blockIdx.x * blockDim.x + threadIdx.x;
    if (i == 0) { frag_first[n_frags] = (int32_t)in.n_reads; fs_first_frag[n_fs] = n_frags; }
    if (i >= in.n_reads) return;
    if (new_frag[i]) frag_first[frag_of[i]] = (int32_t)i;
    if (new_fs[i]) {
        fs_first_frag[fs_of[i]] = frag_of[i];
        const int slot = in.fam_id[i] * 2 + in.fam_strand[i];
        if (atomicCAS(&fam_fs[slot], -1, fs_of[i]) != -1) atomicMax(&T->err, 6);
    }
}
__global__ void __launch_bounds__(256) k_build_frags(UvcPrepIn in, UvcParams P, int32_t rend, const int32_t *endpos, const int32_t *kind, const int32_t *fs_of, const int32_t *dflag_of,
                                                     const int32_t *frag_first, int32_t n_frags, FragRec *frags, int32_t *sweep_flag, int32_t *frag_beg, int32_t *frag_strand, Stage2 *T) {
    int w_span = 0, w_s0 = 0;
    for (int f = blockIdx.x * blockDim.x + threadIdx.x; f < n_frags; f += gridDim.x * blockDim.x) {
    FragRec r; memset(&r, 0, sizeof(r));
    const int a0 = frag_first[f], a1 = frag_first[f + 1];
    r.aln_beg = a0; r.aln_end = a1; r.beg = INT32_MAX; r.end = 0; r.fs = fs_of[a0]; r.strand = in.fam_strand[a0]; r.dflag = dflag_of[a0];
    bool all_simple = true;
    for (int k = a0; k < a1; k++) {
        r.beg = pmin(r.beg, in.pos[k]); r.end = pmax(r.end, endpos[k]) + 1;
        r.normMQ = pmax(r.normMQ, (int)in.mapq[k]);
        all_simple = all_simple && (kind[k] == 0);
    }
    r.end = pmin(r.end, rend);
    const bool amplicon_gated = (((r.dflag & 0x4) || ((P.primerlen > 0) && !(0x2 & P.primer_flag))) && !(P.tn_is_paired && (0x1 & P.primer_flag)));
    r.stat_kind = (all_simple && (a1 - a0) <= 2 && !amplicon_gated) ? 0 : 1;
    sweep_flag[f] = r.stat_kind; frag_beg[f] = r.beg; frag_strand[f] = r.strand;
    frags[f] = r;
    w_span = pmax(w_span, r.end - r.beg); w_s0 += (r.strand == 0);
    }
    __shared__ int sh[4][2];
    w_span = wave_max(w_span); w_s0 = wave_sum(w_s0);
    if ((threadIdx.x & 63) == 0) { sh[threadIdx.x >> 6][0] = w_span; sh[threadIdx.x >> 6][1] = w_s0; }
// ... 135 lines not shown
        if (cigar_off) cigar_off[i] = v[1];
        if (b4_off) b4_off[i] = v[2];
        v[0] += lq[k]; v[1] += nc[k]; v[2] += (lq[k] + 1) >> 1;
    }
}
__global__ void __launch_bounds__(256) k_pack_bq4_reads(const uint8_t *b4, int64_t n_b4, const int64_t *b4_off, const int64_t *seq_off, const int32_t *l_qseq, const uint8_t *quals, int64_t n, int64_t n_bases,
                                                        uint8_t *bases, uint16_t *bq, int32_t *bad) {
    const int sub = threadIdx.x & 15;
    const int64_t grp = ((int64_t)blockIdx.x * blockDim.x + threadIdx.x) >> 4, ngrp = ((int64_t)gridDim.x * blockDim.x) >> 4;
    for (int64_t i = grp; i < n; i += ngrp) {
        const int32_t lq = l_qseq[i];
        const int64_t so = seq_off[i], bo = b4_off[i];
        if (lq < 0 || so < 0 || so + lq > n_bases || bo + ((lq + 1) >> 1) > n_b4) { if (sub == 0) *bad = 1; continue; }
        for (int k = 8 * sub; k < lq; k += 128) {
            if (k + 8 <= lq) {
                uint32_t w; unsigned long long q, bb; uint4 o;
                __builtin_memcpy(&w, b4 + bo + (k >> 1), 4); __builtin_memcpy(&q, quals + so + k, 8);
                unpack8(w, q, bb, o);
                __builtin_memcpy(bases + so + k, &bb, 8); __builtin_memcpy(bq + so + k, &o, 16);
            } else {
                for (int k2 = k; k2 < lq; k2++) {
                    const unsigned byte = b4[bo + (k2 >> 1)];
                    const unsigned b0 = nt16_int((k2 & 1) ? (byte & 15) : (byte >> 4));
                    bases[so + k2] = (uint8_t)b0; bq[so + k2] = (uint16_t)(b0 | (quals[so + k2] << 8));
                }
            }
        }
    }
}
__global__ void __launch_bounds__(256) k_pack_bq4_dense(const uint32_t *b4, const unsigned long long *quals, int64_t n8, unsigned long long *bases, uint4 *bq) {
    for (int64_t i = (int64_t)blockIdx.x * blockDim.x + threadIdx.x; i < n8; i += (int64_t)gridDim.x * blockDim.x) {
        const uint32_t w = b4[i]; const unsigned long long q = quals[i];
        unsigned long long bb; uint4 o;
        unpack8(w, q, bb, o);
        bases[i] = bb;
        bq[i] = o;
    }
}
__global__ void __launch_bounds__(256) k_any_odd(const int32_t *l_qseq, int64_t n, int32_t *bad) {
    int odd = 0;
    for (int64_t i = (int64_t)blockIdx.x * blockDim.x + threadIdx.x; i < n; i += (int64_t)gridDim.x * blockDim.x) odd |= (l_qseq[i] & 1) | (l_qseq[i] < 0);
    if (__any(odd) && (threadIdx.x & 63) == 0) *bad = 1;
}
}
extern "C" size_t uvc_prep_compact_tmp_bytes(int64_t n) { return (size_t)(3 * ((n + SC_TILE - 1) / SC_TILE) + 3) * sizeof(long long) + 64; }
extern "C" int uvc_prep_compact(const int32_t *l_qseq, const int32_t *n_cigar, int64_t n, int64_t n_bases, const uint8_t *bases4, int64_t n_b4, const uint8_t *quals,
                                int64_t *seq_off_out, const int64_t *seq_off_in, int64_t *cigar_off_out, int64_t *b4_off, uint8_t *bases_out, uint16_t *bq_out, int32_t *bad,
                                void *tmp, size_t tmp_bytes, hipStream_t s) {
    hipError_t e = hipSuccess;
    const int ntiles = (int)((n + SC_TILE - 1) / SC_TILE);
    if ((size_t)(3 * ntiles + 3) * sizeof(long long) > tmp_bytes) return (int)hipErrorInvalidValue;
    long long *tile_sums = (long long *)tmp;
    const bool dense_form = bases4 && seq_off_out && 2 * n_b4 == n_bases && (n_bases & 7) == 0 && !(((uintptr_t)bases4) & 3) && !(((uintptr_t)quals | (uintptr_t)bases_out) & 7) && !(((uintptr_t)bq_out) & 15);
    if ((seq_off_out || cigar_off_out || (bases4 && !dense_form)) && n > 0) {
        hipLaunchKernelGGL(k_len_sums, dim3((unsigned)ntiles), dim3(SC_BLOCK), 0, s, l_qseq, n_cigar, n, tile_sums, ntiles);
        hipLaunchKernelGGL(k_tile_tops<3>, dim3(1), dim3(1024), 0, s, tile_sums, ntiles, tile_sums + (size_t)3 * ntiles);
        hipLaunchKernelGGL(k_len_apply, dim3((unsigned)ntiles), dim3(SC_BLOCK), 0, s, l_qseq, n_cigar, n, tile_sums, ntiles, seq_off_out, cigar_off_out, (bases4 && !dense_form) ? b4_off : (int64_t *)nullptr);
    }
    if (e == hipSuccess && bases4) {
        if (dense_form) {
            hipLaunchKernelGGL(k_any_odd, dim3((unsigned)std::min<int64_t>((n + 255) / 256, 4096)), dim3(256), 0, s, l_qseq, n, bad);
            hipLaunchKernelGGL(k_pack_bq4_dense, dim3((unsigned)std::min<int64_t>((n_bases / 8 + 255) / 256 + 1, 16384)), dim3(256), 0, s, (const uint32_t *)bases4, (const unsigned long long *)quals, n_bases / 8,
                               (unsigned long long *)bases_out, (uint4 *)bq_out);
        } else {
            hipLaunchKernelGGL(k_pack_bq4_reads, dim3((unsigned)std::min<int64_t>((n + 15) / 16, 65536)), dim3(256), 0, s, bases4, n_b4, b4_off, seq_off_out ? seq_off_out : seq_off_in, l_qseq, quals, n, n_bases, bases_out, bq_out, bad);
        }
    }
    return (int)e;
}

static inline int pos_bits_of(int64_t npos) { int b = 1; while (((int64_t)1 << b) < npos + 1) b++; return b; }

#define PREP_HIP(call) do { hipError_t e_ = (call); if (e_ != hipSuccess) { snprintf(errmsg, (size_t)errcap, "%s: %s", #call, hipGetErrorString(e_)); return UVCGPU_EDEVICE; } } while (0)

extern "C" int uvc_prep_reads(const UvcPrepIn *inp, const UvcParams *P, int32_t rbeg, int32_t rend, int64_t npos, UvcPrepAlloc alloc, void *ctx, hipStream_t s,
                              UvcPrepOut *out, char *errmsg, int errcap) {
    const UvcPrepIn &in = *inp;
    const int64_t n = in.n_reads;
    memset(out, 0, sizeof(*out));
    errmsg[0] = 0;
    auto A = [&](size_t bytes, int zero) -> void * { return alloc(ctx, std::max<size_t>(bytes, 8), zero); };
#define ALLOC(ptr, T, count, zero) do { ptr = (T *)A(sizeof(T) * (size_t)(count), zero); if (!ptr) { snprintf(errmsg, (size_t)errcap, "hipMalloc(%s)", #ptr); return UVCGPU_ENOMEM; } } while (0)
    const int seg_eligible = (UVC_PLATFORM_IONTORRENT != P->inferred_sequencing_platform) && rbeg >= 65536 && P->bias_thres_interfering_indel <= 10000;
    int32_t *new_frag, *new_fs, *is_complex, *n_p2; int64_t *gaps, *trows, *items, *ins;
    ALLOC(out->endpos, int32_t, n, 0); ALLOC(out->kind, int32_t, n, 0); ALLOC(out->dflag_of, int32_t, n, 0); ALLOC(out->frag_of, int32_t, n, 0); ALLOC(out->fs_of, int32_t, n, 0);
    ALLOC(out->table_off, int64_t, n, 0); ALLOC(out->item_off, int64_t, n, 0); ALLOC(out->gap_off, int64_t, n, 0); ALLOC(out->p2_first, int32_t, n, 0);
    ALLOC(new_frag, int32_t, n, 0); ALLOC(new_fs, int32_t, n, 0); ALLOC(is_complex, int32_t, n, 0); out->is_complex = is_complex; ALLOC(n_p2, int32_t, n, 0); ALLOC(gaps, int64_t, n, 0);
    ALLOC(trows, int64_t, n, 0); ALLOC(items, int64_t, n, 0); ALLOC(ins, int64_t, n, 0);
    Stage1 *dT1; ALLOC(dT1, Stage1, 1, 1);
    Stage2 *dT2; ALLOC(dT2, Stage2, 1, 1);
    const size_t tmp_bytes = (size_t)(3 * ((std::max<int64_t>(n, npos + 2) + SC_TILE - 1) / SC_TILE) + 3) * sizeof(long long) + 64;
    void *tmp; ALLOC(tmp, char, tmp_bytes, 0);
    const int ntiles = (int)((n + SC_TILE - 1) / SC_TILE);
    long long *tile_sums; ALLOC(tile_sums, long long, (size_t)8 * ntiles + 8, 0);
    long long *col_totals = tile_sums + (size_t)8 * ntiles;
    ALLOC(out->complex_ids, int32_t, n, 0);
    hipLaunchKernelGGL(k_read_facts, dim3((unsigned)ntiles), dim3(SC_BLOCK), 0, s, in, rbeg, rend, seg_eligible, out->endpos, out->kind, out->dflag_of, new_frag, new_fs, is_complex, n_p2, gaps, trows, items, ins, dT1, tile_sums, ntiles);
    hipLaunchKernelGGL(k_tile_tops<8>, dim3(1), dim3(1024), 0, s, tile_sums, ntiles, col_totals);
    hipLaunchKernelGGL(k_facts_apply, dim3((unsigned)ntiles), dim3(SC_BLOCK), 0, s, n, tile_sums, ntiles, col_totals, out->kind, new_frag, new_fs, n_p2, trows, items, gaps,
                       out->frag_of, out->fs_of, out->p2_first, out->table_off, out->item_off, out->gap_off, out->complex_ids, dT1);
    auto scan3 = [&](ScanCols C) {
        int64_t nmax = 0; for (int c = 0; c < 3; c++) nmax = std::max(nmax, C.n[c]);
        if (nmax <= 0) return;
        const int nt = (int)((nmax + SC_TILE - 1) / SC_TILE);
        long long *ts = (long long *)tmp;
        hipLaunchKernelGGL(k_cols_sums, dim3((unsigned)nt), dim3(SC_BLOCK), 0, s, C, ts, nt);
        hipLaunchKernelGGL(k_tile_tops<3>, dim3(1), dim3(1024), 0, s, ts, nt, ts + (size_t)3 * nt);
        hipLaunchKernelGGL(k_cols_apply, dim3((unsigned)nt), dim3(SC_BLOCK), 0, s, C, ts, nt);
    };
    auto col = [](ScanCols &C, int c, const void *in, void *out, int64_t n, int in64, int out64, int inclusive) { C.in[c] = in; C.out[c] = out; C.n[c] = n; C.in64[c] = in64; C.out64[c] = out64; C.inclusive[c] = inclusive; };
    Stage1 T1;
    PREP_HIP(hipMemcpyAsync(&T1, dT1, sizeof(T1), hipMemcpyDeviceToHost, s));
    PREP_HIP(hipStreamSynchronize(s));
    if (T1.err) {
        const char *m = T1.err == 1 ? "read offsets out of range" : T1.err == 2 ? "unsupported CIGAR op (process_cigar throws, main_conversion.hpp:902-916)" : T1.err == 3 ? "CIGAR query length != l_qseq"
                      : T1.err == 4 ? "read outside region" : "fam_id / fam_strand out of range";
        snprintf(errmsg, (size_t)errcap, "%s", m);
        return T1.err == 2 ? UVCGPU_EUNSUPPORTED : UVCGPU_EINVAL;
    }
    out->n_frags = T1.n_frags; out->n_fs = T1.n_fs; out->n_complex = T1.n_complex; out->n_simple = (int32_t)(n - T1.n_complex); out->n_p2 = T1.n_p2; out->table_rows = T1.table_rows;
    out->item_slots = T1.item_slots; out->gap_slots = T1.gap_slots; out->ins_total = T1.ins_total; out->max_aln_span = std::max(T1.max_aln_span, 1); out->any_amplicon = T1.any_amplicon;
    out->max_p2_span = std::max(T1.max_p2_span, 1);
    out->p2_off[0] = 0; for (int c = 0; c < 4; c++) out->p2_off[c + 1] = out->p2_off[c] + T1.p2_cls[c];
    const int32_t nf = T1.n_frags, nu = T1.n_fs;
    int32_t *frag_first, *fs_first_frag, *fam_fs, *sweep_flag, *sweep_rank, *generic_flag, *generic_rank, *dup_flag, *dup_rank; int64_t *gen_span, *work_off, *dup_span, *dup_off_all;
    ALLOC(frag_first, int32_t, nf + 1, 0); ALLOC(fs_first_frag, int32_t, nu + 1, 0); ALLOC(fam_fs, int32_t, (size_t)in.n_fams * 2, 0);
    PREP_HIP(hipMemsetAsync(fam_fs, 0xFF, sizeof(int32_t) * std::max<size_t>((size_t)in.n_fams * 2, 1), s));
    ALLOC(sweep_flag, int32_t, nf, 0); ALLOC(sweep_rank, int32_t, nf, 0); ALLOC(generic_flag, int32_t, nu, 0); ALLOC(generic_rank, int32_t, nu, 0); ALLOC(dup_flag, int32_t, nu, 0); ALLOC(dup_rank, int32_t, nu, 0);
    ALLOC(gen_span, int64_t, nu, 0); ALLOC(work_off, int64_t, nu, 0); ALLOC(dup_span, int64_t, nu, 0); ALLOC(dup_off_all, int64_t, nu, 0);
    ALLOC(out->frags, FragRec, nf, 0); ALLOC(out->fss, FsRec, nu, 0); ALLOC(out->frag_beg, int32_t, nf, 0); ALLOC(out->frag_strand, int32_t, nf, 0);
    hipLaunchKernelGGL(k_mark_first, dim3(nblk(n, 256)), dim3(256), 0, s, in, new_frag, new_fs, out->frag_of, out->fs_of, frag_first, fs_first_frag, fam_fs, nf, nu, dT2);
    hipLaunchKernelGGL(k_build_frags, dim3(std::min(nblk(nf, 256), 1024u)), dim3(256), 0, s, in, *P, rend, out->endpos, out->kind, out->fs_of, out->dflag_of, frag_first, nf, out->frags, sweep_flag, out->frag_beg, out->frag_strand, dT2);
    hipLaunchKernelGGL(k_build_units, dim3(nblk(nu, 256)), dim3(256), 0, s, in, *P, rend, out->endpos, out->dflag_of, frag_first, fs_first_frag, fam_fs, nu, out->fss, generic_flag, gen_span, dT2);
    { ScanCols C; memset(&C, 0, sizeof(C)); col(C, 0, generic_flag, generic_rank, nu, 0, 0, 0); col(C, 1, gen_span, work_off, nu, 1, 1, 0); col(C, 2, sweep_flag, sweep_rank, nf, 0, 0, 0); scan3(C); }
    ALLOC(out->generic_fs, int32_t, nu, 0);
    hipLaunchKernelGGL(k_units_post, dim3(nblk(nu, 256)), dim3(256), 0, s, rend, nu, out->fss, generic_rank, work_off, out->generic_fs, dup_flag, dup_span);
    { ScanCols C; memset(&C, 0, sizeof(C)); col(C, 0, dup_flag, dup_rank, nu, 0, 0, 0); col(C, 1, dup_span, dup_off_all, nu, 1, 1, 0); scan3(C); }
    ALLOC(out->dup_units, int32_t, nu, 0); ALLOC(out->dup_off, int64_t, nu, 0);
    hipLaunchKernelGGL(k_compact_dups, dim3(nblk(nu, 256)), dim3(256), 0, s, nu, dup_flag, dup_rank, dup_off_all, out->dup_units, out->dup_off);
    ALLOC(out->sweep_frags, int32_t, nf, 0);
    int32_t *depth = nullptr;
    if (nf >= 65536) { ALLOC(depth, int32_t, npos + 2, 1); }
    hipLaunchKernelGGL(k_frags_post, dim3(nblk(nf, 256)), dim3(256), 0, s, nf, out->frags, out->fss, sweep_flag, sweep_rank, out->sweep_frags, rbeg, depth);
    if (depth) {
        { ScanCols C; memset(&C, 0, sizeof(C)); col(C, 0, depth, depth, npos + 1, 0, 0, 1); scan3(C); }
        hipLaunchKernelGGL(k_max_i32, dim3(256), dim3(256), 0, s, depth, npos + 1, &dT2->max_frag_depth);
    }
    hipLaunchKernelGGL(k_stage2_totals, dim3(1), dim3(1), 0, s, nu, nf, generic_rank, generic_flag, work_off, gen_span, dup_rank, dup_flag, dup_off_all, dup_span, sweep_rank, sweep_flag, dT2);
    const int64_t np2 = T1.n_p2;
    ALLOC(out->p2_aln, int32_t, np2, 0); ALLOC(out->p2_beg, int32_t, np2, 0); ALLOC(out->p2_end, int32_t, np2, 0); ALLOC(out->p2_qb, int32_t, np2, 0); ALLOC(out->p2_cls, int32_t, np2, 0);
    hipLaunchKernelGGL(k_p2_entries, dim3(nblk(n, 256)), dim3(256), 0, s, in, n_p2, out->p2_first, out->p2_aln, out->p2_beg, out->p2_end, out->p2_qb, out->p2_cls);
    Stage2 T2;
    PREP_HIP(hipMemcpyAsync(&T2, dT2, sizeof(T2), hipMemcpyDeviceToHost, s));
    PREP_HIP(hipStreamSynchronize(s));
    if (T2.err) { snprintf(errmsg, (size_t)errcap, "reads of one (fam_id, fam_strand) are not contiguous"); return UVCGPU_EINVAL; }
    out->n_generic = T2.n_generic; out->n_dup = T2.n_dup; out->n_sweep = T2.n_sweep; out->work = T2.work; out->dup_work = T2.dup_work;
    out->max_frag_span = std::max(T2.max_frag_span, 1); out->max_unit_span = std::max(T2.max_unit_span, 1); out->max_unit_frags = T2.max_unit_frags; out->n_frag_strand0 = T2.n_frag_strand0;
    out->max_frag_depth = (nf < 65536 ? nf : T2.max_frag_depth);
    ALLOC(out->generic_sorted, int32_t, std::max(T2.n_generic, 1), 0);
    if (T2.n_generic > 0) {
        const int32_t ng = T2.n_generic;
        int32_t *beg_of, *zero; uint32_t *work; void *stmp;
        const size_t sb = uvc_sort32_tmp_bytes((size_t)ng);
        ALLOC(beg_of, int32_t, ng, 0); ALLOC(zero, int32_t, ng, 0); ALLOC(work, uint32_t, 4 * (size_t)ng, 0); ALLOC(stmp, char, sb + 16, 0);
        hipLaunchKernelGGL(k_unit_keys, dim3(nblk(ng, 256)), dim3(256), 0, s, out->fss, out->generic_fs, ng, beg_of, zero);
        if (uvc_sort_by_pos_cls(beg_of, zero, rbeg, pos_bits_of(npos), 0, ng, work, stmp, sb, s) != 0) { snprintf(errmsg, (size_t)errcap, "device sort of the units failed"); return UVCGPU_EDEVICE; }
        hipLaunchKernelGGL(k_take_units, dim3(nblk(ng, 256)), dim3(256), 0, s, work + 3 * (size_t)ng, out->generic_fs, ng, out->generic_sorted);
    }
    PREP_HIP(hipGetLastError());
    return 0;
#undef ALLOC
}
```

Measured before the change: 109.6 million.

## Merge simple-read FastRec list into the sorted P2 work list

Removes the separate frec array and its dedicated sort of alignments. Simple reads now write their FastRec straight into their slot in the already position/class-sorted P2 list, and the gather kernel records that slot. Non-primary P2 entries are tagged with an M_RUN bit so the pileup sweeps, which now walk the four P2 class lists, skip them where the old list-0 scan would not have seen them. This drops one radix sort, one array and the record copy in build_p2list, at the cost of four smaller window ranges per sweep plus an extra flag check per record.

```diff
diff --git a/uvc_amd/csrc/uvc_device.h b/uvc_amd/csrc/uvc_device.h
--- a/uvc_amd/csrc/uvc_device.h
+++ b/uvc_amd/csrc/uvc_device.h
@@ -45,6 +45,7 @@
     int32_t bmv, xbv, bm4c, clips;
     int32_t baq_pos, baq_last, baq2_last, ext;
 };
+#define FREC_M_RUN (1 << 16)
 
 struct FragRec {
     int32_t aln_beg, aln_end;
@@ -119,7 +120,6 @@
     const uint16_t *bq; uint32_t bq_bytes;
     AlnRec *alns; int32_t n_alns;
     int32_t n_fast;
-    FastRec *frec;
     int32_t p2_off[5];
     FastRec *frec2; int32_t n_fast2; int32_t max_p2_span;
     const int32_t *complex_ids; int32_t n_complex;
@@ -146,7 +146,7 @@
     Item *items; int32_t *item_cnt;
     MisItem *mis; int32_t *mis_cnt; int32_t mis_cap;
     unsigned long long *mis_total;
-    int32_t max_aln_span, max_frag_span;
+    int32_t max_frag_span;
     int32_t any_amplicon;
     int32_t frag32;
     int32_t max_frag_depth;
diff --git a/uvc_amd/csrc/uvc_gap.hip b/uvc_amd/csrc/uvc_gap.hip
--- a/uvc_amd/csrc/uvc_gap.hip
+++ b/uvc_amd/csrc/uvc_gap.hip
@@ -24,11 +24,14 @@
     key[i] = ((uint32_t)(pos[i] - beg) | ((uint32_t)cls[i] << shift)); val[i] = (uint32_t)i;
 }
 __global__ void __launch_bounds__(256) k_gather4(const uint32_t *perm, int64_t n, const int32_t *a0, const int32_t *a1, const int32_t *a2, const int32_t *a3,
-                                                 int32_t *o0, int32_t *o1, int32_t *o2, int32_t *o3) {
+                                                 int32_t *o0, int32_t *o1, int32_t *o2, int32_t *o3, const int32_t *kind, int64_t n_alns, int32_t *slot) {
     const int64_t i = (int64_t)blockIdx.x * blockDim.x + threadIdx.x;
+    if (i < n_alns && kind[i] != 0) slot[i] = -1;
     if (i >= n) return;
     const int64_t j = (int64_t)perm[i];
-    o0[i] = a0[j]; o1[i] = a1[j]; o2[i] = a2[j]; o3[i] = a3[j];
+    const int32_t id = a0[j];
+    o0[i] = id; o1[i] = a1[j]; o2[i] = a2[j]; o3[i] = a3[j];
+    if (kind[id] == 0) slot[id] = (int32_t)i;
 }
 __global__ void __launch_bounds__(256) k_rank_from_sorted(const uint32_t *perm, int64_t n, int64_t n_first, int32_t *out_ids, int32_t *rank) {
     const int64_t k = (int64_t)blockIdx.x * blockDim.x + threadIdx.x;
@@ -50,8 +53,10 @@
     hipLaunchKernelGGL(k_keys_pos_cls, dim3((unsigned)((n + 255) / 256)), dim3(256), 0, s, d_pos, d_cls, beg, pos_bits, n, key, val);
     return rocprim::radix_sort_pairs(tmp, tmp_bytes, key, key_s, val, val_s, (size_t)n, 0, (unsigned)(pos_bits + cls_bits), s) == hipSuccess ? 0 : -1;
 }
-extern "C" void uvc_launch_gather4(const uint32_t *perm, int64_t n, const int32_t *a0, const int32_t *a1, const int32_t *a2, const int32_t *a3, int32_t *o0, int32_t *o1, int32_t *o2, int32_t *o3, hipStream_t s) {
-    if (n > 0) hipLaunchKernelGGL(k_gather4, dim3((unsigned)((n + 255) / 256)), dim3(256), 0, s, perm, n, a0, a1, a2, a3, o0, o1, o2, o3);
+extern "C" void uvc_launch_gather4(const uint32_t *perm, int64_t n, const int32_t *a0, const int32_t *a1, const int32_t *a2, const int32_t *a3, int32_t *o0, int32_t *o1, int32_t *o2, int32_t *o3,
+                                   const int32_t *kind, int64_t n_alns, int32_t *slot, hipStream_t s) {
+    const int64_t m = std::max(n, n_alns);
+    if (m > 0) hipLaunchKernelGGL(k_gather4, dim3((unsigned)((m + 255) / 256)), dim3(256), 0, s, perm, n, a0, a1, a2, a3, o0, o1, o2, o3, kind, n_alns, slot);
 }
 extern "C" void uvc_launch_rank_from_sorted(const uint32_t *perm, int64_t n, int64_t n_first, int32_t *out_ids, int32_t *rank, hipStream_t s) {
     if (n > 0) hipLaunchKernelGGL(k_rank_from_sorted, dim3((unsigned)((n + 255) / 256)), dim3(256), 0, s, perm, n, n_first, out_ids, rank);
diff --git a/uvc_amd/csrc/uvc_host.cpp b/uvc_amd/csrc/uvc_host.cpp
--- a/uvc_amd/csrc/uvc_host.cpp
+++ b/uvc_amd/csrc/uvc_host.cpp
@@ -343,18 +343,14 @@
       uvc_launch_pack_bq(R.bases, R.quals, b, d->n_bases, d_bad, r->stream); }
     { AlnRec *a; if ((rc = dev_alloc(r, (size_t)n, &a))) return rc; R.alns = a; R.n_alns = (int32_t)n; }
     R.n_fast = (int32_t)n_simple;
-    { FastRec *f; if ((rc = dev_alloc(r, (size_t)n_simple, &f))) return rc; R.frec = f; }
     R.complex_ids = o.complex_ids; R.n_complex = o.n_complex;
     R.frags = o.frags; R.n_frags = o.n_frags;
     int pos_bits = 1; while (((int64_t)1 << pos_bits) < r->npos + 1) pos_bits++;
     {
-        const size_t nmax = std::max<size_t>(std::max<size_t>((size_t)n, nf), 1);
-        int32_t *d_rank, *d_fsorted, *d_frank; uint32_t *work; uint8_t *tmp;
+        const size_t nmax = std::max<size_t>(nf, 1);
+        int32_t *d_fsorted, *d_frank; uint32_t *work; uint8_t *tmp;
         const size_t tmp_bytes = uvc_sort32_tmp_bytes(nmax);
-        if ((rc = dev_alloc(r, (size_t)n, &d_rank)) || (rc = dev_alloc(r, nf, &d_fsorted)) || (rc = dev_alloc(r, nf, &d_frank)) || (rc = dev_alloc(r, 4 * nmax, &work)) || (rc = dev_alloc(r, tmp_bytes + 16, &tmp))) return rc;
-        if (uvc_sort_by_pos_cls(W.pos, o.is_complex, r->beg, pos_bits, 1, n, work, tmp, tmp_bytes, r->stream) != 0) return fail(UVCGPU_EDEVICE, "device sort of the alignments failed");
-        uvc_launch_rank_from_sorted(work + 3 * n, n, n_simple, nullptr, d_rank, r->stream);
-        W.fast_rank = d_rank;
+        if ((rc = dev_alloc(r, nf, &d_fsorted)) || (rc = dev_alloc(r, nf, &d_frank)) || (rc = dev_alloc(r, 4 * nmax, &work)) || (rc = dev_alloc(r, tmp_bytes + 16, &tmp))) return rc;
         if (uvc_sort_by_pos_cls(o.frag_beg, o.frag_strand, r->beg, pos_bits, 1, (int64_t)nf, work, tmp, tmp_bytes, r->stream) != 0) return fail(UVCGPU_EDEVICE, "device sort of the fragments failed");
         uvc_launch_rank_from_sorted(work + 3 * nf, (int64_t)nf, (int64_t)nf, d_fsorted, d_frank, r->stream);
         R.frag_sorted = d_fsorted; R.frag_rank = d_frank;
@@ -397,25 +393,26 @@
     }
     { int32_t *c; if ((rc = dev_alloc(r, (size_t)4, &c, true))) return rc; R.mis_cnt = c; R.mis_total = (unsigned long long *)(c + 2); R.mis = nullptr; R.mis_cap = 0; }
     r->d_dup_units = o.dup_units; r->d_dup_off = o.dup_off; r->n_dup = o.n_dup; r->n_dup_work = o.dup_work;
-    R.max_aln_span = o.max_aln_span; R.max_frag_span = o.max_frag_span;
+    R.max_frag_span = o.max_frag_span;
     R.any_amplicon = o.any_amplicon;
     R.max_frag_depth = o.max_frag_depth;
     HIP_OK(hipMemsetAsync(R.table, 0, (size_t)std::max<int64_t>(o.table_rows, 1) * sizeof(Contrib), r->stream));
+    {
+        const size_t np2 = (size_t)o.n_p2;
+        for (int c = 0; c <= 4; c++) R.p2_off[c] = o.p2_off[c];
+        uint32_t *work; uint8_t *tmp; int32_t *d_slot;
+        const size_t tmp_bytes = uvc_sort32_tmp_bytes(std::max<size_t>(np2, 1));
+        if ((rc = dev_alloc(r, 4 * np2, &work)) || (rc = dev_alloc(r, tmp_bytes + 16, &tmp)) || (rc = dev_alloc(r, (size_t)n, &d_slot))) return rc;
+        for (int k = 0; k < 4; k++) if ((rc = dev_alloc(r, np2, &r->d_p2[k]))) return rc;
+        if (uvc_sort_by_pos_cls(o.p2_beg, o.p2_cls, r->beg, pos_bits, 2, (int64_t)np2, work, tmp, tmp_bytes, r->stream) != 0) return fail(UVCGPU_EDEVICE, "device sort of the work list failed");
+        uvc_launch_gather4(work + 3 * np2, (int64_t)np2, o.p2_aln, o.p2_beg, o.p2_end, o.p2_qb, r->d_p2[0], r->d_p2[1], r->d_p2[2], r->d_p2[3], W.kind, n, d_slot, r->stream);
+        W.fast_rank = d_slot;
+        { FastRec *f; if ((rc = dev_alloc(r, np2, &f))) return rc; R.frec2 = f; R.n_fast2 = (int32_t)np2; R.max_p2_span = o.max_p2_span; }
+    }
     lap("allocations + orders");
     uvc_launch_prelude(&R, &W, &r->P, r->stream);
     lap("prelude kernel");
-    {
-        const size_t np2 = (size_t)o.n_p2;
-        for (int c = 0; c <= 4; c++) R.p2_off[c] = o.p2_off[c];
-        uint32_t *work; uint8_t *tmp;
-        const size_t tmp_bytes = uvc_sort32_tmp_bytes(std::max<size_t>(np2, 1));
-        if ((rc = dev_alloc(r, 4 * np2, &work)) || (rc = dev_alloc(r, tmp_bytes + 16, &tmp))) return rc;
-        for (int k = 0; k < 4; k++) if ((rc = dev_alloc(r, np2, &r->d_p2[k]))) return rc;
-        if (uvc_sort_by_pos_cls(o.p2_beg, o.p2_cls, r->beg, pos_bits, 2, (int64_t)np2, work, tmp, tmp_bytes, r->stream) != 0) return fail(UVCGPU_EDEVICE, "device sort of the P2 work list failed");
-        uvc_launch_gather4(work + 3 * np2, (int64_t)np2, o.p2_aln, o.p2_beg, o.p2_end, o.p2_qb, r->d_p2[0], r->d_p2[1], r->d_p2[2], r->d_p2[3], r->stream);
-        { FastRec *f; if ((rc = dev_alloc(r, np2, &f))) return rc; R.frec2 = f; R.n_fast2 = (int32_t)np2; R.max_p2_span = o.max_p2_span; }
-        uvc_launch_build_p2list(&R, W.fast_rank, r->d_p2[0], r->d_p2[1], r->d_p2[2], r->d_p2[3], r->stream);
-    }
+    uvc_launch_build_p2list(&R, W.fast_rank, r->d_p2[0], r->d_p2[1], r->d_p2[2], r->d_p2[3], r->stream);
     HIP_OK(hipGetLastError());
     {
         unsigned long long total = 0; int32_t bad4 = 0;
@@ -429,7 +426,7 @@
         if ((rc = dev_alloc(r, (size_t)(total + 64), &q))) return rc;
         R.mis = q; R.mis_cap = (int32_t)(total + 64);
     }
-    lap("P2 list sort + build");
+    lap("work list build");
     r->n_bases = d->n_bases;
     r->has_reads = true; r->reads_given = true;
     return 0;
diff --git a/uvc_amd/csrc/uvc_kernels_acc.hip b/uvc_amd/csrc/uvc_kernels_acc.hip
--- a/uvc_amd/csrc/uvc_kernels_acc.hip
+++ b/uvc_amd/csrc/uvc_kernels_acc.hip
@@ -41,8 +41,7 @@
     if (t >= per_list * (list_end - list_beg)) return;
     const int list = list_beg + (int)(t / per_list), which = (int)((t % per_list) / R.nwin), w = (int)(t % R.nwin);
     const char *base; int stride, lo, hi, span;
-    if (list == 0) { base = (const char *)&R.frec[0].pos; stride = sizeof(FastRec); lo = 0; hi = R.n_fast; span = R.max_aln_span; }
-    else if (list <= 4) { base = (const char *)&R.frec2[0].pos; stride = sizeof(FastRec); lo = R.p2_off[list - 1]; hi = R.p2_off[list]; span = R.max_p2_span; }
+    if (list <= 4) { base = (const char *)&R.frec2[0].pos; stride = sizeof(FastRec); lo = R.p2_off[list - 1]; hi = R.p2_off[list]; span = R.max_p2_span; }
     else if (list <= 6) { base = (const char *)&R.ffast[0].beg; stride = sizeof(FragFast); lo = R.frag_off[list - 5]; hi = R.frag_off[list - 4]; span = R.max_frag_span; }
     else { base = nullptr; stride = 0; lo = 0; hi = R.n_generic_fs; span = R.max_unit_span; }
     const int w0 = R.beg + 64 * w, key = (which == 0 ? w0 - span + 1 : w0 + 64);
@@ -309,13 +308,13 @@
     return false;
 }
 
-DEV void fill_fastrec(FastRec &f, const AlnRec &a, int id, int cbeg, int cend, int32_t qb_lo) {
+DEV void fill_fastrec(FastRec &f, const AlnRec &a, int id, int cbeg, int cend, int32_t qb_lo, bool m_run) {
     f.pos = cbeg; f.rend = cend; f.qb_lo = qb_lo; f.aln = id;
     f.fmd = (a.flag & 0xFFFF) | ((a.mapq & 0xFF) << 16) | ((a.dflag & 0xFF) << 24); f.isize = a.isize; f.mpos = a.mpos; f.xm1500 = a.xm1500;
     int bv[5];
     for (int s2 = 0; s2 < 5; s2++) bv[s2] = (a.bm1500[s2] > 20 ? (100 * (20 * 20) / (a.bm1500[s2] * a.bm1500[s2])) : 100);
     const int xv = (a.xm1500 > 20 ? (100 * (20 * 20) / (a.xm1500 * a.xm1500)) : 100);
-    f.bmv = bv[0] | (bv[1] << 8) | (bv[2] << 16) | (bv[3] << 24); f.xbv = bv[4] | (xv << 8);
+    f.bmv = bv[0] | (bv[1] << 8) | (bv[2] << 16) | (bv[3] << 24); f.xbv = bv[4] | (xv << 8) | (m_run ? FREC_M_RUN : 0);
     f.bm4c = ((a.clip_cnt & 0xF) << 16) | (a.nogap_penal & 0xFFFF);
     f.clips = (a.lclip_oplen & 0xFFFF) | (a.rclip_oplen << 16);
     f.baq_pos = (int32_t)a.baq_pos; f.baq_last = (int32_t)a.baq_last; f.baq2_last = (int32_t)a.baq2_last;
@@ -325,16 +324,11 @@
 __global__ void __launch_bounds__(256) k_build_p2list(RegionDev R, const int32_t *fast_rank, const int32_t *aln, const int32_t *cbeg, const int32_t *cend, const int32_t *qb) {
     const int j = blockIdx.x * blockDim.x + threadIdx.x;
     if (j >= R.n_fast2) return;
-    const int id = aln[j], rk = fast_rank[id];
-    if (rk >= 0) {
-        const uint4 *src = (const uint4 *)&R.frec[rk]; uint4 *dst = (uint4 *)&R.frec2[j];
-        const uint4 v0 = src[0], v1 = src[1], v2 = src[2], v3 = src[3];
-        dst[0] = v0; dst[1] = v1; dst[2] = v2; dst[3] = v3;
-        return;
-    }
+    const int id = aln[j];
+    if (fast_rank[id] >= 0) return;
     FastRec f;
     const AlnRec &a = R.alns[id];
-    fill_fastrec(f, a, id, cbeg[j], (a.kind == 1 ? cbeg[j] : cend[j]), qb[j]);
+    fill_fastrec(f, a, id, cbeg[j], (a.kind == 1 ? cbeg[j] : cend[j]), qb[j], true);
     R.frec2[j] = f;
 }
 
@@ -363,7 +357,7 @@
 #pragma unroll
         for (int s2 = 0; s2 < 5; s2++) { cnt[s2] += __shfl_xor(cnt[s2], 1); cnt[s2] += __shfl_xor(cnt[s2], 2); cnt[s2] += __shfl_xor(cnt[s2], 4); }
         if (sub == 0) {
-            int32_t *dst = (int32_t *)&R.frec[rk];
+            int32_t *dst = (int32_t *)&R.frec2[rk];
 #pragma unroll
             for (int s2 = 0; s2 < 5; s2++) dst[s2] = cnt[s2];
         }
@@ -393,7 +387,7 @@
     int qpos = 0, rpos = a.pos, lclip_q = 0, m_index = -1;
     const int rk0 = W.fast_rank[id];
     if (rk0 >= 0) {
-        const int32_t *pre = (const int32_t *)&R.frec[rk0];
+        const int32_t *pre = (const int32_t *)&R.frec2[rk0];
         for (int s2 = 0; s2 < 5; s2++) bm[s2] = pre[s2];
         for (int i = 0; i < a.n_cigar && m_index < 0; i++) {
             const int op = cig_op(cigar[i]);
@@ -433,8 +427,8 @@
     if (rk >= 0 || W.kind[id] == 2) n_mis = bm[0] + bm[1] + bm[2] + bm[3] + bm[4];
     if (rk >= 0) {
         FastRec f;
-        fill_fastrec(f, a, id, a.pos, a.rend, (int32_t)(a.qbase & 0xFFFFFFFFLL));
-        R.frec[rk] = f;
+        fill_fastrec(f, a, id, a.pos, a.rend, (int32_t)(a.qbase & 0xFFFFFFFFLL), false);
+        R.frec2[rk] = f;
     }
     return n_mis;
 }
@@ -522,7 +516,6 @@
     for (int i = threadIdx.x; i < 2 * (PSUM_TILE + 1); i += 256) (&d64[0][0])[i] = 0ull;
     __syncthreads();
     const int w_first = (int)blockIdx.x * (PSUM_TILE / 64), w_last = imin(w_first + PSUM_TILE / 64, R.nwin) - 1;
-    const int lo = win_lo(R, 0, w_first), hi = win_hi(R, 0, w_last);
     auto put = [&](int f, int a, int b, int v) {
         a = imax(a, t0); b = imin(b, t1);
         if (a < b && v != 0) { atomicAdd(&d[f][a - t0], v); atomicAdd(&d[f][b - t0], -v); }
@@ -531,11 +524,14 @@
         a = imax(a, t0); b = imin(b, t1);
         if (a < b && v != 0) { atomicAdd(&d64[f][a - t0], (unsigned long long)v); atomicAdd(&d64[f][b - t0], (unsigned long long)(-v)); }
     };
+    for (int cls = 0; cls < 4; cls++) {
+    const int lo = win_lo(R, 1 + cls, w_first), hi = win_hi(R, 1 + cls, w_last);
     for (int k = lo + (int)threadIdx.x; k < hi; k += 256) {
-        const int4 *q4 = (const int4 *)(R.frec + k);
+        const int4 *q4 = (const int4 *)(R.frec2 + k);
         const int4 h0 = q4[0], h1 = q4[1];
         const int apos = h0.x, rend = h0.y;
         if (rend <= t0 || apos >= t1) continue;
+        if (((const int *)q4)[9] & FREC_M_RUN) continue;
         const int dflag = (h1.x >> 24) & 0xFF;
         put(PS_DP, apos, rend, 1); put(PS_PCR, apos, rend, (dflag & 0x4) ? 1 : 0); put(PS_UMI, apos, rend, (dflag & 0x1) ? 1 : 0);
         put(PS_QLEN, apos, rend, rend - apos); put(PS_XM, apos, rend, h1.w);
@@ -552,6 +548,7 @@
                 put64(1, apos, brk, MAX_INSERT_SIZE); put(PS_RIA, brk, rend, 1); put64(1, brk, rend, fr);
             }
         }
+    }
     }
     __syncthreads();
     const int lane = threadIdx.x & 63, w = threadIdx.x >> 6;
@@ -615,7 +612,6 @@
     const int my_baq = valid ? (int)R.baq[x] : 0;
     int ldist = 0, rdist = 0, hbq = 0;
     long long lbaq = 0, rbaq = 0;
-    const int lo = wave_uniform(win_lo(R, 0, (int)(x0 >> 6))), hi = wave_uniform(win_hi(R, 0, (int)(x0 >> 6)));
     COARSE_T(ct1)
     const __amdgpu_buffer_rsrc_t rs = bq_rsrc(R);
     int2 *myq = prepq[threadIdx.x >> 6];
@@ -629,15 +625,18 @@
         }
         nq = 0;
     };
+#pragma unroll 1
+    for (int cls = 0; cls < 4; cls++) {
+    const int lo = wave_uniform(win_lo(R, 1 + cls, (int)(x0 >> 6))), hi = wave_uniform(win_hi(R, 1 + cls, (int)(x0 >> 6)));
     for (int k0 = lo + (SPLIT ? 64 * (int)(threadIdx.x >> 6) : 0); k0 < hi; k0 += (SPLIT ? 256 : 64)) {
         Chunk16 c;
-        load_chunk16(R.frec, k0 + lane, hi, c);
+        load_chunk16(R.frec2, k0 + lane, hi, c);
         const int n = imin(64, hi - k0);
         auto fetch = [&](int j) { return bq_load(rs, bcast(c.v[2], j) + p); };
         auto one = [&](int j, int bqn) {
             const int b = bqn & 0xFF, q = (bqn >> 8) & 0xFF;
             const int apos = bcast(c.v[0], j), rend = bcast(c.v[1], j);
-            if (rend <= w0) return;
+            if (rend <= w0 || (bcast(c.v[9], j) & FREC_M_RUN)) return;
             const bool cover = (valid && p >= apos && p < rend);
             const wmask mm = BAL(cover && b != my_ref);
             if (mm) {
@@ -668,6 +667,7 @@
             if (j + 2 < n) { const int v = r2; if (j + 6 < n) r2 = fetch(j + 6); one(j + 2, v); }
             if (j + 3 < n) { const int v = r3; if (j + 7 < n) r3 = fetch(j + 7); one(j + 3, v); }
         }
+    }
     }
     if (nq > 0) drain();
     COARSE_T(ct2)
@@ -3355,8 +3355,8 @@
     hipStream_t s2 = (side ? side : s);
     hipStream_t s3 = ((side && side3) ? side3 : s2);
     {
-        const int64_t n = 2 * (int64_t)R->nwin * 5;
-        TIMED(prof, "k_win_index", hipLaunchKernelGGL(k_win_index, dim3(nblk(n, 256)), dim3(256), 0, s, *R, 0, 5));
+        const int64_t n = 2 * (int64_t)R->nwin * 4;
+        TIMED(prof, "k_win_index", hipLaunchKernelGGL(k_win_index, dim3(nblk(n, 256)), dim3(256), 0, s, *R, 1, 5));
         if (R->n_generic_fs) hipLaunchKernelGGL(k_win_index, dim3(nblk(2 * (int64_t)R->nwin, 256)), dim3(256), 0, s, *R, 7, 8);
     }
     if (P->inferred_is_vcf_generated && R->n_fast) TIMED(prof, "k_prep_sums", hipLaunchKernelGGL(k_prep_sums, dim3(nblk(R->npos, PSUM_TILE)), dim3(256), 0, s, *R, *P));
diff --git a/uvc_amd/csrc/uvc_launch.h b/uvc_amd/csrc/uvc_launch.h
--- a/uvc_amd/csrc/uvc_launch.h
+++ b/uvc_amd/csrc/uvc_launch.h
@@ -90,7 +90,8 @@
 int uvc_gap_sort(void *tmp, size_t tmp_bytes, const unsigned long long *kin, unsigned long long *kout, const unsigned long long *vin, unsigned long long *vout, size_t n, int end_bit, hipStream_t s);
 size_t uvc_sort32_tmp_bytes(size_t n);
 int uvc_sort_by_pos_cls(const int32_t *d_pos, const int32_t *d_cls, int32_t beg, int pos_bits, int cls_bits, int64_t n, uint32_t *work , void *tmp, size_t tmp_bytes, hipStream_t s);
-void uvc_launch_gather4(const uint32_t *perm, int64_t n, const int32_t *a0, const int32_t *a1, const int32_t *a2, const int32_t *a3, int32_t *o0, int32_t *o1, int32_t *o2, int32_t *o3, hipStream_t s);
+void uvc_launch_gather4(const uint32_t *perm, int64_t n, const int32_t *a0, const int32_t *a1, const int32_t *a2, const int32_t *a3, int32_t *o0, int32_t *o1, int32_t *o2, int32_t *o3,
+                        const int32_t *kind, int64_t n_alns, int32_t *slot, hipStream_t s);
 void uvc_launch_rank_from_sorted(const uint32_t *perm, int64_t n, int64_t n_first, int32_t *out_ids, int32_t *rank, hipStream_t s);
 void uvc_launch_gather_columns(const char *const *base, const int32_t *first_col, const int32_t *elem, int64_t npos, const int32_t *d_xs, int64_t n, long long *d_out, hipStream_t s);
 size_t uvc_prep_compact_tmp_bytes(int64_t n);
diff --git a/uvc_amd/csrc/uvc_prep.h b/uvc_amd/csrc/uvc_prep.h
--- a/uvc_amd/csrc/uvc_prep.h
+++ b/uvc_amd/csrc/uvc_prep.h
@@ -10,14 +10,14 @@
     const uint32_t *cigars;
 };
 struct UvcPrepOut {
-    int32_t *endpos, *kind, *dflag_of, *frag_of, *fs_of, *p2_first, *complex_ids, *is_complex;
+    int32_t *endpos, *kind, *dflag_of, *frag_of, *fs_of, *p2_first, *complex_ids;
     int32_t *frag_beg, *frag_strand;
     int64_t *table_off, *item_off, *gap_off;
     FragRec *frags; FsRec *fss;
     int32_t *generic_fs, *generic_sorted, *sweep_frags, *dup_units; int64_t *dup_off;
     int32_t *p2_aln, *p2_beg, *p2_end, *p2_qb, *p2_cls;
     int32_t n_frags, n_fs, n_complex, n_simple, n_generic, n_dup, n_sweep, n_frag_strand0;
-    int32_t max_aln_span, max_frag_span, max_unit_span, max_unit_frags, max_p2_span, max_frag_depth, any_amplicon;
+    int32_t max_frag_span, max_unit_span, max_unit_frags, max_p2_span, max_frag_depth, any_amplicon;
     int32_t p2_off[5];
     int64_t n_p2, table_rows, item_slots, gap_slots, ins_total, work, dup_work;
 };
diff --git a/uvc_amd/csrc/uvc_prep.hip b/uvc_amd/csrc/uvc_prep.hip
--- a/uvc_amd/csrc/uvc_prep.hip
+++ b/uvc_amd/csrc/uvc_prep.hip
@@ -101,7 +101,7 @@
 }
 
 struct Stage1 {
-    int32_t err, max_aln_span, n_frags, n_fs, n_complex, any_amplicon;
+    int32_t err, n_frags, n_fs, n_complex, any_amplicon, pad0_;
     int32_t p2_cls[4]; int32_t max_p2_span, pad_;
     int64_t n_p2, table_rows, item_slots, gap_slots, ins_total;
 };
@@ -111,9 +111,9 @@
 };
 
 __global__ void __launch_bounds__(256) k_read_facts(UvcPrepIn in, int32_t rbeg, int32_t rend, int seg_eligible,
-                                                    int32_t *endpos, int32_t *kind, int32_t *dflag_of, int32_t *new_frag, int32_t *new_fs, int32_t *is_complex,
+                                                    int32_t *endpos, int32_t *kind, int32_t *dflag_of, int32_t *new_frag, int32_t *new_fs,
                                                     int32_t *n_p2, int64_t *gaps, int64_t *trows, int64_t *items, int64_t *ins, Stage1 *T, long long *tile_sums, int ntiles) {
-    int w_err = 0, w_span = 0, w_p2span = 0, w_cls[4] = { 0, 0, 0, 0 }, w_amp = 0;
+    int w_err = 0, w_p2span = 0, w_cls[4] = { 0, 0, 0, 0 }, w_amp = 0;
     long long col[8] = { 0, 0, 0, 0, 0, 0, 0, 0 };
     for (int k8 = 0; k8 < SC_ITEMS; k8++) {
     const int64_t i = (int64_t)blockIdx.x * SC_TILE + (int64_t)k8 * SC_BLOCK + threadIdx.x;
@@ -161,7 +161,7 @@
             o_end = e; o_np2 = (ok ? np2 : 0);
             o_kind = simple ? 0 : (ok ? 2 : 1);
             if (!simple) { o_trows = (e - pos) + 1; o_items = 2 * (int64_t)lq + 2 * del_total + nc + 4; }
-            else { o_gaps = 0; o_ins = 0; w_span = pmax(w_span, e - pos); }
+            else { o_gaps = 0; o_ins = 0; }
             if (o_np2) {
                 const int fl = in.flag[i];
                 const int cls = ((fl & 0x10) ? 1 : 0) | ((((fl & 0x81) == 0x81) ? ((fl & 0x20) != 0) : ((fl & 0x10) != 0)) ? 2 : 0);
@@ -170,7 +170,7 @@
         }
     }
     if (err) { w_err = pmax(w_err, err); o_kind = 1; o_gaps = 0; o_ins = 0; o_np2 = 0; }
-    endpos[i] = o_end; kind[i] = o_kind; n_p2[i] = o_np2; gaps[i] = o_gaps; trows[i] = o_trows; items[i] = o_items; ins[i] = o_ins; is_complex[i] = (o_kind != 0);
+    endpos[i] = o_end; kind[i] = o_kind; n_p2[i] = o_np2; gaps[i] = o_gaps; trows[i] = o_trows; items[i] = o_items; ins[i] = o_ins;
     const bool ok_fam = !bad_fam;
     const int df = ok_fam ? (int)in.fam_dflag[fam] : 0;
     dflag_of[i] = df;
@@ -185,20 +185,19 @@
         block_sums<8>(col, shc);
         if (threadIdx.x == 0) { for (int c = 0; c < 8; c++) tile_sums[(size_t)c * ntiles + blockIdx.x] = col[c]; }
     }
-    __shared__ int sh[4][8];
-    w_err = wave_max(w_err); w_span = wave_max(w_span); w_p2span = wave_max(w_p2span); w_amp = wave_max(w_amp);
+    __shared__ int sh[4][7];
+    w_err = wave_max(w_err); w_p2span = wave_max(w_p2span); w_amp = wave_max(w_amp);
     for (int c = 0; c < 4; c++) w_cls[c] = wave_sum(w_cls[c]);
     const int wv = threadIdx.x >> 6;
-    if ((threadIdx.x & 63) == 0) { sh[wv][0] = w_err; sh[wv][1] = w_span; sh[wv][2] = w_p2span; sh[wv][3] = w_amp; for (int c = 0; c < 4; c++) sh[wv][4 + c] = w_cls[c]; }
+    if ((threadIdx.x & 63) == 0) { sh[wv][0] = w_err; sh[wv][1] = w_p2span; sh[wv][2] = w_amp; for (int c = 0; c < 4; c++) sh[wv][3 + c] = w_cls[c]; }
     __syncthreads();
     if (threadIdx.x == 0) {
-        int v[8];
-        for (int q = 0; q < 8; q++) { v[q] = sh[0][q]; for (int w = 1; w < 4; w++) v[q] = (q < 4 ? pmax(v[q], sh[w][q]) : v[q] + sh[w][q]); }
+        int v[7];
+        for (int q = 0; q < 7; q++) { v[q] = sh[0][q]; for (int w = 1; w < 4; w++) v[q] = (q < 3 ? pmax(v[q], sh[w][q]) : v[q] + sh[w][q]); }
         if (v[0]) atomicMax(&T->err, v[0]);
-        if (v[1]) atomicMax(&T->max_aln_span, v[1]);
-        if (v[2]) atomicMax(&T->max_p2_span, v[2]);
-        if (v[3]) T->any_amplicon = 1;
-        for (int c = 0; c < 4; c++) if (v[4 + c]) atomicAdd(&T->p2_cls[c], v[4 + c]);
+        if (v[1]) atomicMax(&T->max_p2_span, v[1]);
+        if (v[2]) T->any_amplicon = 1;
+        for (int c = 0; c < 4; c++) if (v[3 + c]) atomicAdd(&T->p2_cls[c], v[3 + c]);
     }
 }
 
@@ -500,10 +499,10 @@
     auto A = [&](size_t bytes, int zero) -> void * { return alloc(ctx, std::max<size_t>(bytes, 8), zero); };
 #define ALLOC(ptr, T, count, zero) do { ptr = (T *)A(sizeof(T) * (size_t)(count), zero); if (!ptr) { snprintf(errmsg, (size_t)errcap, "hipMalloc(%s)", #ptr); return UVCGPU_ENOMEM; } } while (0)
     const int seg_eligible = (UVC_PLATFORM_IONTORRENT != P->inferred_sequencing_platform) && rbeg >= 65536 && P->bias_thres_interfering_indel <= 10000;
-    int32_t *new_frag, *new_fs, *is_complex, *n_p2; int64_t *gaps, *trows, *items, *ins;
+    int32_t *new_frag, *new_fs, *n_p2; int64_t *gaps, *trows, *items, *ins;
     ALLOC(out->endpos, int32_t, n, 0); ALLOC(out->kind, int32_t, n, 0); ALLOC(out->dflag_of, int32_t, n, 0); ALLOC(out->frag_of, int32_t, n, 0); ALLOC(out->fs_of, int32_t, n, 0);
     ALLOC(out->table_off, int64_t, n, 0); ALLOC(out->item_off, int64_t, n, 0); ALLOC(out->gap_off, int64_t, n, 0); ALLOC(out->p2_first, int32_t, n, 0);
-    ALLOC(new_frag, int32_t, n, 0); ALLOC(new_fs, int32_t, n, 0); ALLOC(is_complex, int32_t, n, 0); out->is_complex = is_complex; ALLOC(n_p2, int32_t, n, 0); ALLOC(gaps, int64_t, n, 0);
+    ALLOC(new_frag, int32_t, n, 0); ALLOC(new_fs, int32_t, n, 0); ALLOC(n_p2, int32_t, n, 0); ALLOC(gaps, int64_t, n, 0);
     ALLOC(trows, int64_t, n, 0); ALLOC(items, int64_t, n, 0); ALLOC(ins, int64_t, n, 0);
     Stage1 *dT1; ALLOC(dT1, Stage1, 1, 1);
     Stage2 *dT2; ALLOC(dT2, Stage2, 1, 1);
@@ -513,7 +512,7 @@
     long long *tile_sums; ALLOC(tile_sums, long long, (size_t)8 * ntiles + 8, 0);
     long long *col_totals = tile_sums + (size_t)8 * ntiles;
     ALLOC(out->complex_ids, int32_t, n, 0);
-    hipLaunchKernelGGL(k_read_facts, dim3((unsigned)ntiles), dim3(SC_BLOCK), 0, s, in, rbeg, rend, seg_eligible, out->endpos, out->kind, out->dflag_of, new_frag, new_fs, is_complex, n_p2, gaps, trows, items, ins, dT1, tile_sums, ntiles);
+    hipLaunchKernelGGL(k_read_facts, dim3((unsigned)ntiles), dim3(SC_BLOCK), 0, s, in, rbeg, rend, seg_eligible, out->endpos, out->kind, out->dflag_of, new_frag, new_fs, n_p2, gaps, trows, items, ins, dT1, tile_sums, ntiles);
     hipLaunchKernelGGL(k_tile_tops<8>, dim3(1), dim3(1024), 0, s, tile_sums, ntiles, col_totals);
     hipLaunchKernelGGL(k_facts_apply, dim3((unsigned)ntiles), dim3(SC_BLOCK), 0, s, n, tile_sums, ntiles, col_totals, out->kind, new_frag, new_fs, n_p2, trows, items, gaps,
                        out->frag_of, out->fs_of, out->p2_first, out->table_off, out->item_off, out->gap_off, out->complex_ids, dT1);
@@ -537,7 +536,7 @@
         return T1.err == 2 ? UVCGPU_EUNSUPPORTED : UVCGPU_EINVAL;
     }
     out->n_frags = T1.n_frags; out->n_fs = T1.n_fs; out->n_complex = T1.n_complex; out->n_simple = (int32_t)(n - T1.n_complex); out->n_p2 = T1.n_p2; out->table_rows = T1.table_rows;
-    out->item_slots = T1.item_slots; out->gap_slots = T1.gap_slots; out->ins_total = T1.ins_total; out->max_aln_span = std::max(T1.max_aln_span, 1); out->any_amplicon = T1.any_amplicon;
+    out->item_slots = T1.item_slots; out->gap_slots = T1.gap_slots; out->ins_total = T1.ins_total; out->any_amplicon = T1.any_amplicon;
     out->max_p2_span = std::max(T1.max_p2_span, 1);
     out->p2_off[0] = 0; for (int c = 0; c < 4; c++) out->p2_off[c + 1] = out->p2_off[c] + T1.p2_cls[c];
     const int32_t nf = T1.n_frags, nu = T1.n_fs;
```

Measured after the change: 112.2 million, median of 6. +2.4%, better.
